# bjing2016/mdgen

Measured on AMD Instinct MI355X. Metric: sampled MD frames/sec, higher is better.
Workload: dtype bf16

## Files before the change

### mdgen_amd/csrc/api.hip

```cpp
#include "../../include/mdgen_amd.h"
#include "kernels.h"
#include "linear.h"

#include <algorithm>
#include <cmath>
#include <cstdarg>
#include <cstdio>
#include <cstdlib>
#include <cstring>
#include <climits>
#include <functional>
#include <map>
#include <string>
#include <vector>

using namespace mdg;

static thread_local char g_err[512] = "";
static int fail(int code, const char* fmt, ...) {
    va_list ap;
    va_start(ap, fmt);
    vsnprintf(g_err, sizeof(g_err), fmt, ap);
    va_end(ap);
    return code;
}
struct DryPlan {
    int view = -1;
    std::vector<std::pair<int, const char*>> rec;
};
static thread_local DryPlan* g_dry = nullptr;
#define HIPCHK(expr)                                                                           \
    do {                                                                                       \
        if (g_dry) break;                                                                      \
        hipError_t e_ = (expr);                                                                \
        if (e_ != hipSuccess) return fail((int)e_, "%s failed: %s", #expr, hipGetErrorString(e_)); \
    } while (0)
#define LAUNCHCHK()                                                                            \
    do {                                                                                       \
        hipError_t e_ = hipGetLastError();                                                     \
        if (e_ != hipSuccess) return fail((int)e_, "kernel launch failed: %s (%s:%d)", hipGetErrorString(e_), __FILE__, __LINE__); \
        if (const char* m_ = k32_take_launch_error()) return fail(-7, "internal: %s (%s:%d)", m_, __FILE__, __LINE__); \
    } while (0)

extern "C" const char* mdgen_last_error(void) { return g_err; }
extern "C" int32_t mdgen_abi_version(void) { return MDGEN_ABI_VERSION; }
extern "C" int32_t mdgen_dev_build(void) {
#ifdef MDGEN_DEV_BUILD
    return 1;
#else
    return 0;
#endif
}

constexpr int kMaxPos = 8160;
constexpr int kKS = 24;
constexpr size_t kPackCC = (size_t)12 * kKS * 64;

struct Lin { int w = -1, b = -1; };
struct MhaW {
    bf16x8 *wq = nullptr, *wk = nullptr, *wv_flash = nullptr, *wv_small = nullptr, *wo = nullptr;
    float *bq = nullptr, *bk = nullptr, *bv_flash = nullptr, *bv_small = nullptr, *bo = nullptr;
    float *bias_k = nullptr, *bias_v = nullptr;
    struct { Lin q, k, v, o; int bias_k = -1, bias_v = -1; } slot;
};
struct FfnW {
    bf16x8 *w1 = nullptr, *w2 = nullptr;
    float *b1 = nullptr, *b2 = nullptr;
    bf16x8* wstream = nullptr;
    float* w2f = nullptr;
    struct { Lin fc1, fc2; } slot;
};
struct TrunkW {
    MhaW mha_l, mha_t;
    FfnW ffn;
    Lin ada;
};
struct IpaW {
    float* gamma_beta = nullptr;
    bf16x8* wproj = nullptr;
    float* bproj = nullptr;
    float* head_w = nullptr;
    bf16x8* wout = nullptr;
    float* bout = nullptr;
    MhaW mha_l;
    FfnW ffn;
    struct { Lin ada, norm, q, kv, q_points, kv_points, out; int head_w = -1; } slot;
};

struct ProfRec {
    const char* cls;
    hipEvent_t a, b;
};

struct GraphEntry {
    std::vector<uint64_t> key;
    hipGraph_t graph = nullptr;
    hipGraphExec_t exec = nullptr;
};

struct WeightSlot {
    std::string name;
    std::function<int(const float*, const int64_t*, int, hipStream_t)> set;
    bool provided = false;
    float* f32 = nullptr;
    bool bound = false;
};

struct mdgen_ctx {
    mdgen_model_desc d;
    int nl = 0, D = 0, modrow = 0;
    std::vector<void*> allocs;
    std::vector<WeightSlot> weights;
    std::map<std::string, int> slot_of;
    struct { Lin latent, cond, t0, t2, rel_f, rel_r, fin, fin_ada; int mask = -1, aatype = -1; } slot;
    bool finalized = false;
    float *wl = nullptr, *bl = nullptr, *wc = nullptr, *bc = nullptr, *mask_emb = nullptr, *aa_emb = nullptr;
    float *wl_pack = nullptr, *wc_pack = nullptr;
    float* mask_delta = nullptr;
    bf16x8 *wl_hi = nullptr, *wl_lo = nullptr, *wc_hi = nullptr, *wc_lo = nullptr;
    float *pos_embed = nullptr, *t_w0 = nullptr, *t_b0 = nullptr, *t_w2 = nullptr, *t_b2 = nullptr;
    float *wf7 = nullptr, *bf7 = nullptr, *wr7 = nullptr, *br7 = nullptr;
    float *ada_w = nullptr, *ada_b = nullptr;
    float *inv_freq = nullptr, *rope = nullptr;
    bf16x8* wfin = nullptr;
    bf16x8* wfin_k = nullptr;
    float* bfin = nullptr;
    std::vector<TrunkW> trunk;
    std::vector<IpaW> ipa;
    int *map_nat = nullptr, *map_qk = nullptr, *map_vflash = nullptr, *map_vsmall = nullptr, *map_fin = nullptr;
    int *perm_qk = nullptr, *perm_vsmall = nullptr;
    int* mlp_tab = nullptr;
    std::vector<GraphEntry> graphs;
    bool inv_freq_set = false;
    bool prof_on = false;
    int opt_precision = 16;
    int opt_keep_fp32 = 0;
    int opt_streams = 2;
    bool opt_streams_auto = true;
    int opt_attn_path = 0;
    int opt_mlp_path = 1;
    int opt_fuse_proj_qkv = 1;
    int opt_fuse_proj = 3;
    int opt_panel_waves = 0;
    int ncu = 256;
    int opt_small_split = 1;
    bool xcd_round_robin = false;
    long n_split_launches = 0;
    int opt_flash_rotate = 1;
    int opt_flash_proj_form = 0;
    int opt_flash_proj = 1;
    int opt_train_precision = 32;
    int opt_train_streams = 2;
    hipStream_t train_side = nullptr;
    struct TurnReq { const float* w[3]; int nseg, rows, cols; size_t off; };
    std::vector<TurnReq> tr_plan;
    float* tr_buf = nullptr;
    size_t tr_buf_floats = 0;
    bool tr_plan_ok = false;
    std::vector<hipEvent_t> train_ev;
    size_t train_ev_next = 0;
    double* ode_host = nullptr;
    int opt_mlp_fold = 1;
    int opt_mlp_tail = 2;
    int opt_residue_l4 = 2;
    std::vector<void*> milestone_events;
    unsigned long long* phase_trace = nullptr;
    long phase_trace_cap = 0;
    std::vector<ProfRec> prof;
    static constexpr int kMaxSide = 7;
    hipStream_t side[kMaxSide] = {};
    hipEvent_t ev_fork = nullptr, ev_join[kMaxSide] = {};

    const float* f32(int slot) const { return weights[slot].f32; }
    bool any_f32() const {
        return std::any_of(weights.begin(), weights.end(), [](const WeightSlot& w) { return w.f32 != nullptr; });
    }
    template <typename T>
    int dalloc(T** p, size_t count) {
        void* q = nullptr;
        hipError_t e = hipMalloc(&q, count * sizeof(T));
        if (e != hipSuccess) return fail((int)e, "hipMalloc(%zu) failed: %s", count * sizeof(T), hipGetErrorString(e));
        allocs.push_back(q);
        *p = (T*)q;
        return 0;
    }
    int trunk_off(int i) const { return i * 9 * kC; }
    int ipa_off(int i) const { return nl * 9 * kC + i * 6 * kC; }
    int final_off() const { return nl * 15 * kC; }
};

static void decode_T(int rho, int& hd, int& h, int& e) {
    const int ft = rho / 32, m = rho % 32;
    const int b = m & 3, hh = (m >> 2) & 1, a = m >> 3;
    const int ap = 4 * ft + a;
    hd = ap / 3;
    h = hh;
    e = 4 * (ap % 3) + b;
}
static int feat_qk(int w, int rho) {
    int hd, h, e;
    decode_T(rho, hd, h, e);
    return (4 * w + hd) * kDH + 6 * h + (e >> 1) + 12 * (e & 1);
}
static int feat_vsmall(int w, int rho) {
    int hd, h, e;
    decode_T(rho, hd, h, e);
    return (4 * w + hd) * kDH + 12 * h + e;
}
static int feat_vflash(int w, int col) {
    const int hd = col / kDH, d = col % kDH;
    return (4 * w + hd) * kDH + 12 * ((d >> 2) & 1) + 4 * (d >> 3) + (d & 3);
}

static void build_maps(std::vector<int>& qk, std::vector<int>& vf, std::vector<int>& vs, std::vector<int>& pqk,
                       std::vector<int>& pvs) {
    qk.assign(kC, 0); vf.assign(kC, 0); vs.assign(kC, 0); pqk.assign(kC, 0); pvs.assign(kC, 0);
    for (int w = 0; w < 4; ++w)
        for (int r = 0; r < 96; ++r) {
            qk[w * 96 + r] = feat_qk(w, r);
            vs[w * 96 + r] = feat_vsmall(w, r);
            vf[w * 96 + r] = feat_vflash(w, r);
        }
    for (int w = 0; w < 4; ++w)
        for (int h = 0; h < 2; ++h)
            for (int hd = 0; hd < 4; ++hd)
                for (int e = 0; e < 12; ++e) {
                    const int i = ((w * 2 + h) * 4 + hd) * 12 + e;
                    pqk[i] = (4 * w + hd) * kDH + 6 * h + (e >> 1) + 12 * (e & 1);
                    pvs[i] = (4 * w + hd) * kDH + 12 * h + e;
                }
}

extern "C" int32_t mdgen_debug_layout_maps(int32_t* map_qk, int32_t* map_vflash, int32_t* map_vsmall,
                                           int32_t* perm_qk, int32_t* perm_vsmall) {
    if (!map_qk || !map_vflash || !map_vsmall || !perm_qk || !perm_vsmall) return fail(-1, "null argument");
    std::vector<int> qk, vf, vs, pqk, pvs;
    build_maps(qk, vf, vs, pqk, pvs);
    for (int i = 0; i < kC; ++i) {
        map_qk[i] = qk[i]; map_vflash[i] = vf[i]; map_vsmall[i] = vs[i]; perm_qk[i] = pqk[i]; perm_vsmall[i] = pvs[i];
    }
    return 0;
}

static std::vector<int> mlp_stream_table() {
    std::vector<int> t;
    auto xblock = [&](int c, int kx) {
        for (int q = 0; q < 12; ++q) t.push_back(0 << 16 | (2 * c + (q & 1)) << 8 | (6 * kx + (q >> 1)));
    };
    auto yblock = [&](int c, int kk) {
        for (int ft = 0; ft < 12; ++ft) t.push_back(1 << 16 | ft << 8 | (4 * c + kk));
    };
    for (int c = 0; c < 2; ++c)
        for (int kx = 0; kx < 4; ++kx) xblock(c, kx);
    for (int c = 1; c < 23; ++c)
        for (int b = 0; b < 4; ++b) {
            xblock(c + 1, b);
            yblock(c - 1, b);
        }
    for (int c = 22; c < 24; ++c)
        for (int kk = 0; kk < 4; ++kk) yblock(c, kk);
    return t;
}
constexpr int kMlpFrags = 2304;
extern "C" int32_t mdgen_debug_mlp_stream_table(int32_t* out, int32_t capacity) {
    const std::vector<int> t = mlp_stream_table();
    if (!out || capacity < (int)t.size()) return fail(-1, "need room for %d entries", (int)t.size());
    for (size_t i = 0; i < t.size(); ++i) out[i] = t[i];
    return (int32_t)t.size();
}

static int upload_ints(mdgen_ctx* c, int** dst, const std::vector<int>& v) {
    if (int r = c->dalloc(dst, v.size())) return r;
    HIPCHK(hipMemcpy(*dst, v.data(), v.size() * sizeof(int), hipMemcpyHostToDevice));
    return 0;
}

static bool shape_is(const int64_t* s, int nd, std::initializer_list<int64_t> want) {
    std::vector<int64_t> a(s, s + nd), b(want);
    while (a.size() > b.size() && a.front() == 1) a.erase(a.begin());
    return a == b;
}

static int add_weight(mdgen_ctx* c, const std::string& key, std::function<int(const float*, const int64_t*, int, hipStream_t)> set) {
    c->slot_of[key] = (int)c->weights.size();
    c->weights.push_back(WeightSlot{key, std::move(set)});
    return (int)c->weights.size() - 1;
}
#define SETTER(key, body)                                                                          \
    add_weight(c, key, [=](const float* data, const int64_t* shp, int nd, hipStream_t s) -> int {  \
        (void)shp; (void)nd; body; return 0; })
#define WANT(...) \
    if (!shape_is(shp, nd, {__VA_ARGS__})) return fail(-3, "unexpected shape for weight")

static int copy_f32(float* dst, const float* src, size_t n, hipStream_t s) {
    HIPCHK(hipMemcpyAsync(dst, src, n * sizeof(float), hipMemcpyDeviceToDevice, s));
    return 0;
}

static int register_mha(mdgen_ctx* c, const std::string& pre, MhaW* m) {
    const float qscale = (1.0f / std::sqrt((float)kDH)) * kLog2e;
    if (int r = c->dalloc(&m->wq, kPackCC)) return r;
    if (int r = c->dalloc(&m->wk, kPackCC)) return r;
    if (int r = c->dalloc(&m->wv_flash, kPackCC)) return r;
    if (int r = c->dalloc(&m->wv_small, kPackCC)) return r;
    if (int r = c->dalloc(&m->wo, kPackCC)) return r;
    for (float** p : {&m->bq, &m->bk, &m->bv_flash, &m->bv_small, &m->bo, &m->bias_k, &m->bias_v})
        if (int r = c->dalloc(p, (size_t)kC)) return r;
    m->slot.q.w = SETTER(pre + "q_proj.weight", {
        WANT(kC, kC);
        launch_pack_rows(data, kC, c->map_qk, 12, kKS, qscale, m->wq, s);
    });
    m->slot.q.b = SETTER(pre + "q_proj.bias", { WANT(kC); launch_gather_f32(data, c->perm_qk, qscale, m->bq, kC, s); });
    m->slot.k.w = SETTER(pre + "k_proj.weight", {
        WANT(kC, kC);
        launch_pack_rows(data, kC, c->map_qk, 12, kKS, 1.f, m->wk, s);
    });
    m->slot.k.b = SETTER(pre + "k_proj.bias", { WANT(kC); launch_gather_f32(data, c->perm_qk, 1.f, m->bk, kC, s); });
    m->slot.v.w = SETTER(pre + "v_proj.weight", {
        WANT(kC, kC);
        launch_pack_rows(data, kC, c->map_vflash, 12, kKS, 1.f, m->wv_flash, s);
        launch_pack_rows(data, kC, c->map_vsmall, 12, kKS, 1.f, m->wv_small, s);
    });
    m->slot.v.b = SETTER(pre + "v_proj.bias", {
        WANT(kC);
        launch_gather_f32(data, c->map_vflash, 1.f, m->bv_flash, kC, s);
        launch_gather_f32(data, c->perm_vsmall, 1.f, m->bv_small, kC, s);
    });
    m->slot.o.w = SETTER(pre + "out_proj.weight", {
        WANT(kC, kC);
        launch_pack_rows(data, kC, c->map_nat, 12, kKS, 1.f, m->wo, s);
    });
    m->slot.o.b = SETTER(pre + "out_proj.bias", { WANT(kC); if (int r = copy_f32(m->bo, data, kC, s)) return r; });
    m->slot.bias_k = SETTER(pre + "bias_k", { WANT(kC); if (int r = copy_f32(m->bias_k, data, kC, s)) return r; });
    m->slot.bias_v = SETTER(pre + "bias_v", { WANT(kC); if (int r = copy_f32(m->bias_v, data, kC, s)) return r; });
    SETTER(pre + "rot_emb.inv_freq", {
        WANT(12);
        if (int r = copy_f32(c->inv_freq, data, 12, s)) return r;
        c->inv_freq_set = true;
    });
    return 0;
}

static int register_ffn(mdgen_ctx* c, const std::string& pre, FfnW* f, bool trunk) {
    if (trunk)
        if (int r = c->dalloc(&f->w2f, (size_t)kC * kF)) return r;
    if (int r = c->dalloc(&f->w1, (size_t)48 * kKS * 64)) return r;
    if (int r = c->dalloc(&f->w2, (size_t)12 * 96 * 64)) return r;
    if (int r = c->dalloc(&f->b1, (size_t)kF)) return r;
    if (int r = c->dalloc(&f->b2, (size_t)kC)) return r;
    if (int r = c->dalloc(&f->wstream, (size_t)kMlpFrags * 64)) return r;
    f->slot.fc1.w = SETTER(pre + "fc1.weight", {
        WANT(kF, kC);
        launch_pack_rows(data, kC, c->map_nat, 48, kKS, 1.f, f->w1, s);
        launch_pack_stream(data, kC, 0, c->mlp_tab, kMlpFrags, 1.f, 1, f->wstream, s);
    });
    f->slot.fc1.b = SETTER(pre + "fc1.bias", { WANT(kF); if (int r = copy_f32(f->b1, data, kF, s)) return r; });
    f->slot.fc2.w = SETTER(pre + "fc2.weight", {
        WANT(kC, kF);
        launch_pack_rows(data, kF, c->map_nat, 12, 96, 1.f, f->w2, s);
        launch_pack_stream(data, kF, 1, c->mlp_tab, kMlpFrags, 1.f, 1, f->wstream, s);
        if (f->w2f)
            if (int r = copy_f32(f->w2f, data, (size_t)kC * kF, s)) return r;
    });
    f->slot.fc2.b = SETTER(pre + "fc2.bias", { WANT(kC); if (int r = copy_f32(f->b2, data, kC, s)) return r; });
    return 0;
}

extern "C" int32_t mdgen_ctx_create(mdgen_ctx** out, const mdgen_model_desc* d) {
    if (!out || !d) return fail(-1, "null argument");
    if (d->embed_dim != kC || d->mha_heads != kH) return fail(-2, "this build supports embed_dim=384, mha_heads=16 only");
    if (d->ipa_heads != 4 || d->ipa_head_dim != 32 || d->ipa_qk != 8 || d->ipa_v != 8)
        return fail(-2, "this build supports ipa_heads=4, ipa_head_dim=32, ipa_qk=ipa_v=8 only");
    if (d->num_layers < 1 || d->num_layers > 8) return fail(-2, "num_layers must be in 1..8");
    if (d->latent_dim != 21 && d->latent_dim != 28)
        return fail(-2, "latent_dim must be 21 (forward simulation) or 28 (two-sided conditioning)");
    if (d->tps_condition && d->latent_dim != 28) return fail(-2, "tps_condition requires latent_dim 28");
    int ndev = 0;
    HIPCHK(hipGetDeviceCount(&ndev));
    if (ndev < 1) return fail(-9, "no HIP device");
    mdgen_ctx* c = new mdgen_ctx();
    {
        int dev = 0, ncu = 0;
        if (hipGetDevice(&dev) == hipSuccess && hipDeviceGetAttribute(&ncu, hipDeviceAttributeMultiprocessorCount, dev) == hipSuccess && ncu > 0)
            c->ncu = ncu;
    }
    {
        int* dp = nullptr;
        int hx[64];
        hipStream_t ps = nullptr;
        if (hipStreamCreateWithFlags(&ps, hipStreamNonBlocking) == hipSuccess) {
            if (hipMalloc((void**)&dp, sizeof(hx)) == hipSuccess) {
                launch_xcc_probe(dp, 64, ps);
                if (hipGetLastError() == hipSuccess &&
                    hipMemcpyAsync(hx, dp, sizeof(hx), hipMemcpyDeviceToHost, ps) == hipSuccess &&
                    hipStreamSynchronize(ps) == hipSuccess) {
                    bool ok = true;
                    for (int i = 8; i < 64; ++i) ok = ok && hx[i] == hx[i & 7];
                    c->xcd_round_robin = ok;
                }
                (void)hipFree(dp);
            }
            (void)hipStreamDestroy(ps);
        }
        (void)hipGetLastError();
    }
    c->d = *d;
    c->nl = d->num_layers;
    c->D = d->latent_dim;
    c->modrow = (15 * c->nl + 2) * kC;
    const int D = c->D, nl = c->nl;
    std::vector<int> nat(kF), qk, vf, vs, fin(32), pqk, pvs;
    for (int i = 0; i < kF; ++i) nat[i] = i;
    build_maps(qk, vf, vs, pqk, pvs);
    for (int i = 0; i < 32; ++i) fin[i] = i < D ? i : -1;
#define TRY(x) do { if (int r_ = (x)) { mdgen_ctx_destroy(c); return r_; } } while (0)
    TRY(upload_ints(c, &c->map_nat, nat));
    TRY(upload_ints(c, &c->map_qk, qk));
    TRY(upload_ints(c, &c->map_vflash, vf));
    TRY(upload_ints(c, &c->map_vsmall, vs));
    TRY(upload_ints(c, &c->map_fin, fin));
    TRY(upload_ints(c, &c->mlp_tab, mlp_stream_table()));
    TRY(upload_ints(c, &c->perm_qk, pqk));
    TRY(upload_ints(c, &c->perm_vsmall, pvs));
    TRY(c->dalloc(&c->wl, (size_t)kC * D));
    TRY(c->dalloc(&c->wl_pack, (size_t)kEmbPackFloats));
    TRY(c->dalloc(&c->wc_pack, (size_t)kEmbPackFloats));
    TRY(c->dalloc(&c->mask_delta, (size_t)kC));
    for (bf16x8** q : {&c->wl_hi, &c->wl_lo, &c->wc_hi, &c->wc_lo}) TRY(c->dalloc(q, (size_t)12 * 2 * 64));
    TRY(c->dalloc(&c->bl, (size_t)kC));
    TRY(c->dalloc(&c->wc, (size_t)kC * D));
    TRY(c->dalloc(&c->bc, (size_t)kC));
    TRY(c->dalloc(&c->mask_emb, (size_t)2 * kC));
    TRY(c->dalloc(&c->aa_emb, (size_t)21 * kC));
    TRY(c->dalloc(&c->t_w0, (size_t)kC * 256));
    TRY(c->dalloc(&c->t_b0, (size_t)kC));
    TRY(c->dalloc(&c->t_w2, (size_t)kC * kC));
    TRY(c->dalloc(&c->t_b2, (size_t)kC));
    TRY(c->dalloc(&c->ada_w, (size_t)c->modrow * kC));
    TRY(c->dalloc(&c->ada_b, (size_t)c->modrow));
    TRY(c->dalloc(&c->inv_freq, (size_t)12));
    TRY(c->dalloc(&c->rope, (size_t)(kMaxPos + 1) * kRopeRow));
#define TRYHIP(expr)                                                                                    \
    do {                                                                                                \
        hipError_t e_ = (expr);                                                                         \
        if (e_ != hipSuccess) {                                                                         \
            mdgen_ctx_destroy(c);                                                                       \
            return fail((int)e_, "%s failed: %s", #expr, hipGetErrorString(e_));                        \
        }                                                                                               \
    } while (0)
    for (int i = 0; i < mdgen_ctx::kMaxSide; ++i) {
        TRYHIP(hipStreamCreateWithFlags(&c->side[i], hipStreamNonBlocking));
        TRYHIP(hipEventCreateWithFlags(&c->ev_join[i], hipEventDisableTiming));
    }
    TRYHIP(hipEventCreateWithFlags(&c->ev_fork, hipEventDisableTiming));
    TRY(c->dalloc(&c->wfin, (size_t)kKS * 64));
    TRY(c->dalloc(&c->wfin_k, (size_t)kKS * 64));
    TRY(c->dalloc(&c->bfin, (size_t)32));
    TRYHIP(hipMemset(c->bfin, 0, 32 * sizeof(float)));
#undef TRYHIP
    c->slot.latent.w = SETTER("latent_to_emb.weight", { WANT(kC, c->D); if (int r = copy_f32(c->wl, data, (size_t)kC * c->D, s)) return r; launch_pack_embed(c->wl, c->D, c->wl_pack, s);
        launch_pack_rows(c->wl, c->D, c->map_nat, 12, 2, 1.f, c->wl_hi, s, 1, 0); launch_pack_rows(c->wl, c->D, c->map_nat, 12, 2, 1.f, c->wl_lo, s, 1, 1); });
    c->slot.latent.b = SETTER("latent_to_emb.bias", { WANT(kC); if (int r = copy_f32(c->bl, data, kC, s)) return r; });
    c->slot.cond.w = SETTER("cond_to_emb.weight", { WANT(kC, c->D); if (int r = copy_f32(c->wc, data, (size_t)kC * c->D, s)) return r; launch_pack_embed(c->wc, c->D, c->wc_pack, s);
        launch_pack_rows(c->wc, c->D, c->map_nat, 12, 2, 1.f, c->wc_hi, s, 1, 0); launch_pack_rows(c->wc, c->D, c->map_nat, 12, 2, 1.f, c->wc_lo, s, 1, 1); });
    c->slot.cond.b = SETTER("cond_to_emb.bias", { WANT(kC); if (int r = copy_f32(c->bc, data, kC, s)) return r; });
    c->slot.mask = SETTER("mask_to_emb.weight", { WANT(2, kC); if (int r = copy_f32(c->mask_emb, data, 2 * kC, s)) return r; launch_sub_f32(c->mask_emb + kC, c->mask_emb, c->mask_delta, kC, s); });
    c->slot.aatype = SETTER("aatype_to_emb.weight", { WANT(21, kC); if (int r = copy_f32(c->aa_emb, data, 21 * kC, s)) return r; });
    c->slot.t0.w = SETTER("t_embedder.mlp.0.weight", { WANT(kC, 256); if (int r = copy_f32(c->t_w0, data, (size_t)kC * 256, s)) return r; });
    c->slot.t0.b = SETTER("t_embedder.mlp.0.bias", { WANT(kC); if (int r = copy_f32(c->t_b0, data, kC, s)) return r; });
    c->slot.t2.w = SETTER("t_embedder.mlp.2.weight", { WANT(kC, kC); if (int r = copy_f32(c->t_w2, data, (size_t)kC * kC, s)) return r; });
    c->slot.t2.b = SETTER("t_embedder.mlp.2.bias", { WANT(kC); if (int r = copy_f32(c->t_b2, data, kC, s)) return r; });
    if (d->abs_pos_emb) {
        if (d->crop < 1) { mdgen_ctx_destroy(c); return fail(-2, "abs_pos_emb requires crop >= 1"); }
        TRY(c->dalloc(&c->pos_embed, (size_t)d->crop * kC));
        SETTER("pos_embed", { WANT(c->d.crop, kC); if (int r = copy_f32(c->pos_embed, data, (size_t)c->d.crop * kC, s)) return r; });
    }
    if (d->tps_condition) {
        TRY(c->dalloc(&c->wf7, (size_t)kC * 7));
        TRY(c->dalloc(&c->bf7, (size_t)kC));
        TRY(c->dalloc(&c->wr7, (size_t)kC * 7));
        TRY(c->dalloc(&c->br7, (size_t)kC));
        c->slot.rel_f.w = SETTER("latent_to_emb_f.weight", { WANT(kC, 7); if (int r = copy_f32(c->wf7, data, kC * 7, s)) return r; });
        c->slot.rel_f.b = SETTER("latent_to_emb_f.bias", { WANT(kC); if (int r = copy_f32(c->bf7, data, kC, s)) return r; });
        c->slot.rel_r.w = SETTER("latent_to_emb_r.weight", { WANT(kC, 7); if (int r = copy_f32(c->wr7, data, kC * 7, s)) return r; });
        c->slot.rel_r.b = SETTER("latent_to_emb_r.bias", { WANT(kC); if (int r = copy_f32(c->br7, data, kC, s)) return r; });
    }
    c->slot.fin.w = SETTER("emb_to_latent.linear.weight",
           { WANT(c->D, kC); launch_pack_rows(data, kC, c->map_fin, 1, kKS, 1.f, c->wfin, s); launch_pack_rows(data, kC, c->map_fin, 1, kKS, 1.f, c->wfin_k, s, 1); });
    c->slot.fin.b = SETTER("emb_to_latent.linear.bias", { WANT(c->D); if (int r = copy_f32(c->bfin, data, c->D, s)) return r; });
    c->slot.fin_ada.w = SETTER("emb_to_latent.adaLN_modulation.1.weight", {
        WANT(2 * kC, kC);
        if (int r = copy_f32(c->ada_w + (size_t)c->final_off() * kC, data, (size_t)2 * kC * kC, s)) return r;
    });
    c->slot.fin_ada.b = SETTER("emb_to_latent.adaLN_modulation.1.bias",
           { WANT(2 * kC); if (int r = copy_f32(c->ada_b + c->final_off(), data, 2 * kC, s)) return r; });
    c->trunk.resize(nl);
    c->ipa.resize(nl);
    for (int i = 0; i < nl; ++i) {
        const std::string p = "layers." + std::to_string(i) + ".";
        TrunkW* t = &c->trunk[i];
        t->ada.w = SETTER(p + "adaLN_modulation.1.weight", {
            WANT(9 * kC, kC);
            if (int r = copy_f32(c->ada_w + (size_t)c->trunk_off(i) * kC, data, (size_t)9 * kC * kC, s)) return r;
        });
        t->ada.b = SETTER(p + "adaLN_modulation.1.bias",
               { WANT(9 * kC); if (int r = copy_f32(c->ada_b + c->trunk_off(i), data, 9 * kC, s)) return r; });
        TRY(register_mha(c, p + "mha_t.attn.", &t->mha_t));
        TRY(register_mha(c, p + "mha_l.attn.", &t->mha_l));
        TRY(register_ffn(c, p, &t->ffn, true));
    }
    for (int i = 0; i < nl; ++i) {
        const std::string p = "ipa_layers." + std::to_string(i) + ".";
        IpaW* w = &c->ipa[i];
        TRY(c->dalloc(&w->gamma_beta, (size_t)2 * kC));
        TRY(c->dalloc(&w->wproj, (size_t)21 * kKS * 64));
        TRY(c->dalloc(&w->bproj, (size_t)kIpaProj));
        TRY(c->dalloc(&w->head_w, (size_t)4));
        TRY(c->dalloc(&w->wout, (size_t)12 * 16 * 64));
        TRY(c->dalloc(&w->bout, (size_t)kC));
        w->slot.ada.w = SETTER(p + "adaLN_modulation.1.weight", {
            WANT(6 * kC, kC);
            if (int r = copy_f32(c->ada_w + (size_t)c->ipa_off(i) * kC, data, (size_t)6 * kC * kC, s)) return r;
        });
        w->slot.ada.b = SETTER(p + "adaLN_modulation.1.bias",
               { WANT(6 * kC); if (int r = copy_f32(c->ada_b + c->ipa_off(i), data, 6 * kC, s)) return r; });
        w->slot.norm.w = SETTER(p + "ipa_norm.weight", { WANT(kC); if (int r = copy_f32(w->gamma_beta, data, kC, s)) return r; });
        w->slot.norm.b = SETTER(p + "ipa_norm.bias", { WANT(kC); if (int r = copy_f32(w->gamma_beta + kC, data, kC, s)) return r; });
        w->slot.head_w = SETTER(p + "ipa.head_weights", { WANT(4); if (int r = copy_f32(w->head_w, data, 4, s)) return r; });
        w->slot.q.w = SETTER(p + "ipa.linear_q.weight", { WANT(128, kC); launch_pack_rows(data, kC, c->map_nat, 4, kKS, 1.f, w->wproj, s); });
        w->slot.q.b = SETTER(p + "ipa.linear_q.bias", { WANT(128); if (int r = copy_f32(w->bproj, data, 128, s)) return r; });
        w->slot.kv.w = SETTER(p + "ipa.linear_kv.weight",
               { WANT(256, kC); launch_pack_rows(data, kC, c->map_nat, 8, kKS, 1.f, w->wproj + (size_t)4 * kKS * 64, s); });
        w->slot.kv.b = SETTER(p + "ipa.linear_kv.bias", { WANT(256); if (int r = copy_f32(w->bproj + 128, data, 256, s)) return r; });
        w->slot.q_points.w = SETTER(p + "ipa.linear_q_points.weight",
               { WANT(96, kC); launch_pack_rows(data, kC, c->map_nat, 3, kKS, 1.f, w->wproj + (size_t)12 * kKS * 64, s); });
        w->slot.q_points.b = SETTER(p + "ipa.linear_q_points.bias", { WANT(96); if (int r = copy_f32(w->bproj + 384, data, 96, s)) return r; });
        w->slot.kv_points.w = SETTER(p + "ipa.linear_kv_points.weight",
               { WANT(192, kC); launch_pack_rows(data, kC, c->map_nat, 6, kKS, 1.f, w->wproj + (size_t)15 * kKS * 64, s); });
        w->slot.kv_points.b = SETTER(p + "ipa.linear_kv_points.bias", { WANT(192); if (int r = copy_f32(w->bproj + 480, data, 192, s)) return r; });
        w->slot.out.w = SETTER(p + "ipa.linear_out.weight",
               { WANT(kC, kIpaFeat); launch_pack_rows(data, kIpaFeat, c->map_nat, 12, 16, 1.f, w->wout, s); });
        w->slot.out.b = SETTER(p + "ipa.linear_out.bias", { WANT(kC); if (int r = copy_f32(w->bout, data, kC, s)) return r; });
        TRY(register_mha(c, p + "mha_l.attn.", &w->mha_l));
        TRY(register_ffn(c, p, &w->ffn, false));
    }
#undef TRY
    *out = c;
    return 0;
}

extern "C" int32_t mdgen_ctx_destroy(mdgen_ctx* c) {
    if (!c) return 0;
    for (auto& g : c->graphs) {
        if (g.exec) (void)hipGraphExecDestroy(g.exec);
        if (g.graph) (void)hipGraphDestroy(g.graph);
    }
    if (c->ev_fork) (void)hipEventDestroy(c->ev_fork);
    for (hipEvent_t e : c->train_ev) (void)hipEventDestroy(e);
    if (c->train_side) (void)hipStreamDestroy(c->train_side);
    if (c->tr_buf) (void)hipFree(c->tr_buf);
    if (c->ode_host) (void)hipHostFree(c->ode_host);
    for (int i = 0; i < mdgen_ctx::kMaxSide; ++i) {
        if (c->ev_join[i]) (void)hipEventDestroy(c->ev_join[i]);
        if (c->side[i]) (void)hipStreamDestroy(c->side[i]);
    }
    for (void* p : c->allocs) (void)hipFree(p);
    delete c;
    return 0;
}

extern "C" int32_t mdgen_ctx_num_weights(const mdgen_ctx* c) { return c ? (int32_t)c->weights.size() : 0; }
extern "C" const char* mdgen_ctx_weight_name(const mdgen_ctx* c, int32_t i) {
    if (!c || i < 0 || i >= (int32_t)c->weights.size()) return nullptr;
    return c->weights[i].name.c_str();
}

extern "C" int32_t mdgen_ctx_set_weight(mdgen_ctx* c, const char* key, const float* data, const int64_t* shape,
                                        int32_t ndim, void* stream) {
    if (!c || !key || !data || !shape) return fail(-1, "null argument");
    auto it = c->slot_of.find(key);
    if (it == c->slot_of.end()) return fail(-4, "unknown weight key '%s'", key);
    WeightSlot& w = c->weights[it->second];
    const int r = w.set(data, shape, ndim, (hipStream_t)stream);
    if (r) {
        if (r == -3) {
            char buf[160] = "";
            int o = 0;
            for (int i = 0; i < ndim && o < 140; ++i) o += snprintf(buf + o, sizeof(buf) - o, "%lld,", (long long)shape[i]);
            return fail(-3, "unexpected shape (%s) for weight '%s'", buf, key);
        }
        return r;
    }
    LAUNCHCHK();
    if (c->opt_keep_fp32) {
        size_t n = 1;
        for (int i = 0; i < ndim; ++i) n *= (size_t)shape[i];
        if (!w.f32)
            if (int e = c->dalloc(&w.f32, n)) return e;
        if (w.f32 != data && !w.bound)
            HIPCHK(hipMemcpyAsync(w.f32, data, n * sizeof(float), hipMemcpyDeviceToDevice, (hipStream_t)stream));
    }
    w.provided = true;
    c->finalized = false;
    return 0;
}

extern "C" int32_t mdgen_ctx_finalize(mdgen_ctx* c, void* stream) {
    if (!c) return fail(-1, "null context");
    for (const WeightSlot& w : c->weights)
        if (!w.provided) return fail(-5, "weight '%s' was not provided", w.name.c_str());
    if (!c->inv_freq_set) return fail(-5, "rot_emb.inv_freq was not provided");
    launch_rope_table(c->rope, c->inv_freq, kMaxPos + 1, (hipStream_t)stream);
    LAUNCHCHK();
    c->finalized = true;
    return 0;
}

extern "C" int32_t mdgen_ctx_set_option(mdgen_ctx* c, const char* name, int32_t value) {
    if (!c || !name) return fail(-1, "null argument");
    const std::string n(name);
    if (n == "streams") {
        if (value < 1 || value > mdgen_ctx::kMaxSide + 1) return fail(-2, "streams must be in 1..%d", mdgen_ctx::kMaxSide + 1);
        c->opt_streams = value;
        c->opt_streams_auto = false;
    } else if (n == "keep_fp32_weights") {
        if (value != 0 && value != 1) return fail(-2, "keep_fp32_weights must be 0 or 1");
        c->opt_keep_fp32 = value;
    } else if (n == "precision") {
        if (value != 16 && value != 32) return fail(-2, "precision must be 16 (bf16 operands) or 32 (fp32 operands)");
        if (value == 32 && (!c->opt_keep_fp32 || !c->any_f32()))
            return fail(-6, "precision 32 needs the fp32 weight copies: set option keep_fp32_weights = 1 before loading weights");
        c->opt_precision = value;
    } else if (n == "attention_path") {
        if (value != 0 && value != 1) return fail(-2, "attention_path must be 0 (auto) or 1 (robust loop always)");
        c->opt_attn_path = value;
    } else if (n == "fuse_proj") {
        if (value != 0 && value != 3) return fail(-2, "fuse_proj must be 0 (off) or 3 (inside the panel MLP kernel where that kernel runs)");
        c->opt_fuse_proj = value;
    } else if (n == "fuse_proj_qkv") {
        if (value != 0 && value != 1) return fail(-2, "fuse_proj_qkv must be 0 or 1");
        c->opt_fuse_proj_qkv = value;
    } else if (n == "small_split") {
        if (value != 0 && value != 1) return fail(-2, "small_split must be 0 or 1");
        c->opt_small_split = value;
    } else if (n == "panel_waves") {
        if (value != 0 && value != 4 && value != 8) return fail(-2, "panel_waves must be 0 (by launch size), 4 or 8");
        c->opt_panel_waves = value;
    } else if (n == "flash_rotate") {
        if (value != 0 && value != 1) return fail(-2, "flash_rotate must be 0 or 1");
        c->opt_flash_rotate = value;
    } else if (n == "flash_proj_form") {
        if (value != 0 && value != 4 && value != 8) return fail(-2, "flash_proj_form must be 0 (by shape), 4 or 8");
        c->opt_flash_proj_form = value;
    } else if (n == "flash_proj") {
        if (value < 0 || value > 2) return fail(-2, "flash_proj must be 0 (off), 1 (launches that fill the chip) or 2 (always)");
        c->opt_flash_proj = value;
    } else if (n == "mlp_path") {
        if (value < 0 || value > 2) return fail(-2, "mlp_path must be 0 (panel kernel), 1 (row-owner kernel when it fills the chip) or 2 (always)");
        c->opt_mlp_path = value;
    } else if (n == "train_precision") {
        if (value != 16 && value != 32) return fail(-2, "train_precision must be 32 (fp32 operands, exact) or 16 (bf16 operands, fp32 accumulate)");
        c->opt_train_precision = value;
    } else if (n == "train_streams") {
        if (value != 1 && value != 2) return fail(-2, "train_streams must be 1 (one stream) or 2 (weight gradients on a second stream)");
        c->opt_train_streams = value;
    } else if (n == "mlp_fold") {
        if (value != 0 && value != 1) return fail(-2, "mlp_fold must be 0 or 1");
        c->opt_mlp_fold = value;
    } else if (n == "mlp_tail") {
        if (value < 0 || value > 2) return fail(-2, "mlp_tail must be 0 (off), 1 (FinalLayer + Euler update) or 2 (... + the next step's token embedding)");
        c->opt_mlp_tail = value;
    } else if (n == "residue_l4_path") {
        if (value < 0 || value > 2) return fail(-2, "residue_l4_path must be 0, 1 or 2");
        c->opt_residue_l4 = value;
    } else {
        return fail(-4, "unknown option '%s'", name);
    }
    return 0;
}

static size_t align256(size_t x) { return (x + 255) & ~(size_t)255; }

static long split_panels(const mdgen_ctx* c, long maxrows) {
    if (!c->opt_small_split) return 0;
    const long pn = (maxrows + kPanel - 1) / kPanel, cap = c->ncu / kMlpSplit < kMlpSplitMaxPanels ? c->ncu / kMlpSplit : kMlpSplitMaxPanels;
    return pn < cap ? pn : cap;
}
constexpr size_t kSplitCounterBytes = 1024;
static_assert(kMlpSplitMaxPanels * sizeof(unsigned) <= kSplitCounterBytes, "counter block");
static size_t split_bytes(long panels) { return kSplitCounterBytes + 2 * (size_t)panels * kMlpSplit * kPanel * kC * 4; }

static bool mlp_uses_rows(const mdgen_ctx* c, long nrows) {
    const long tiles = (nrows + 31) / 32;
    return c->opt_mlp_path == 2 || (c->opt_mlp_path == 1 && tiles >= 3L * c->ncu);
}
constexpr size_t kFoldStreamBytes = (size_t)kMlpFrags * 1024;
constexpr size_t kFoldMaxBytes = (size_t)8 << 30;
static size_t fold_bytes(const mdgen_ctx* c, int S) { return (size_t)S * c->nl * (kFoldStreamBytes + (size_t)kC * 4); }
static bool fold_on(const mdgen_ctx* c, long nrows, int t_shared, int S) {
    return t_shared && c->opt_mlp_fold && c->opt_precision == 16 && mlp_uses_rows(c, nrows) && fold_bytes(c, S) <= kFoldMaxBytes;
}
static bool embed_base_on(const mdgen_ctx* c, long nrows, int t_shared, int S) {
    return fold_on(c, nrows, t_shared, S) && c->opt_mlp_tail == 2 && S > 1;
}

static size_t frag_bytes(long nseq, int len) { return (size_t)nseq * kH * (len / 32 + 1) * kFragBytes; }

constexpr long kMaxViewTokens = 0xFFFFFFFFL / (kC * 4);

static int plan_views(long B, long T, long L, int streams) {
    const long tl = T * L;
    if (tl > kMaxViewTokens) return 0;
    const long per = kMaxViewTokens / tl;
    long nv = (B + per - 1) / per;
    if (nv < streams) nv = streams;
    if (nv > B) nv = B;
    while ((B + nv - 1) / nv > per) ++nv;
    return (int)nv;
}

extern "C" int32_t mdgen_debug_view_plan(const mdgen_shape* sh, int32_t streams, int32_t* n_views,
                                         int32_t* max_batch_per_view) {
    if (!sh || !n_views || !max_batch_per_view) return fail(-1, "null argument");
    if (sh->B < 1 || sh->T < 1 || sh->L < 1 || streams < 1) return fail(-2, "B, T, L, streams must be >= 1");
    const int nv = plan_views(sh->B, sh->T, sh->L, streams);
    if (nv == 0) return fail(-2, "one sample (T*L = %ld tokens) exceeds the per-launch limit of %ld tokens",
                             (long)sh->T * sh->L, kMaxViewTokens);
    *n_views = nv;
    *max_batch_per_view = (sh->B + nv - 1) / nv;
    return 0;
}

static int check_shape(const mdgen_ctx* c, const mdgen_shape* sh, int S) {
    if (!c || !sh) return fail(-1, "null argument");
    if (sh->B < 1 || sh->T < 1 || sh->L < 1 || S < 1) return fail(-2, "B, T, L, n_steps must be >= 1");
    if (sh->T > kMaxPos - 1 || sh->L > kMaxPos - 1) return fail(-2, "T and L must be < %d", kMaxPos - 1);
    if ((long)sh->B * sh->T * sh->L > 1500000000L) return fail(-2, "token count too large");
    if ((long)sh->T * sh->L > kMaxViewTokens)
        return fail(-2, "one sample (T*L = %ld tokens) exceeds the per-launch limit of %ld tokens", (long)sh->T * sh->L,
                    kMaxViewTokens);
    if ((long)S * sh->B * sh->L > kMaxViewTokens)
        return fail(-2, "n_steps*B*L = %ld rows of the IPA table exceed the per-launch limit of %ld", (long)S * sh->B * sh->L,
                    kMaxViewTokens);
    if (c->d.abs_pos_emb && sh->L > c->d.crop) return fail(-2, "L=%d exceeds pos_embed crop=%d", sh->L, c->d.crop);
    return 0;
}

extern "C" int32_t mdgen_workspace_layout(const mdgen_ctx* c, const mdgen_shape* sh, int32_t S, int32_t t_shared,
                                          mdgen_ws_layout* o) {
    if (!o) return fail(-1, "null argument");
    if (int r = check_shape(c, sh, S)) return r;
    const long B = sh->B, T = sh->T, L = sh->L;
    const long N = B * T * L, Mp = (long)S * B * L, R = t_shared ? S : (long)S * B;
    const long maxrows = N > Mp ? N : Mp;
    size_t fq = (size_t)maxrows * 3 * kC * 2;
    size_t fkv = 0;
    auto upd = [&](size_t b) { if (b > fq) fq = b; if (b > fkv) fkv = b; };
    upd(frag_bytes(B * L, (int)T));
    if (L > 8) {
        upd(frag_bytes(B * T, (int)L));
        upd(frag_bytes((long)S * B, (int)L));
    }
    if (fkv == 0) fkv = 256;
    size_t off = 0;
    auto take = [&](size_t bytes) { size_t a = off; off += align256(bytes); return a; };
// ... 232 lines not shown
    switch (f) {
    case MlpPanelForm::W4: return trunk ? "mlp@p4" : "ipa.mlp@p4";
    case MlpPanelForm::W8: return trunk ? "mlp@p8" : "ipa.mlp@p8";
    case MlpPanelForm::W8Split: return trunk ? "mlp@p8x3" : "ipa.mlp@p8x3";
    case MlpPanelForm::PreW4: return trunk ? "proj_mlp@p4" : "ipa.mlp@p4";
    case MlpPanelForm::PreW8: return trunk ? "proj_mlp@p8" : "ipa.mlp@p8";
    case MlpPanelForm::PreW8Split: return trunk ? "proj_mlp@p8x3" : "ipa.mlp@p8x3";
    }
    return nullptr;
}

static int panel_waves_for(const mdgen_ctx* c, long panels) {
    return c->opt_panel_waves == 4 || c->opt_panel_waves == 8 ? c->opt_panel_waves : (panels <= c->ncu ? 8 : 4);
}
static QkvForm qkv_form(const mdgen_ctx* c, const AxisMap& ax) {
    const long panels = (long)ax.nseq * ((ax.len + kPanel - 1) / kPanel);
    if (panel_waves_for(c, panels) != 8) return QkvForm::Panel4;
    if (!c->opt_small_split || 2 * panels > c->ncu) return QkvForm::Panel8;
    return 2L * ax.nseq * ((ax.len + 31) / 32) <= c->ncu ? QkvForm::Panel8SplitHalf : QkvForm::Panel8Split;
}
static Attn4Form attn4_fused_form(const mdgen_ctx* c, long nrows) {
#ifdef MDGEN_DEV_ATTN4_FULL
    return Attn4Form::Fused;
#else
    return c->opt_small_split && (nrows + 31) / 32 <= c->ncu ? Attn4Form::FusedHalf : Attn4Form::Fused;
#endif
}
static bool flash_proj_on(const mdgen_ctx* c, const AxisMap& ax) {
    return c->opt_precision == 16 && (c->opt_flash_proj == 2 || (c->opt_flash_proj == 1 && flash_proj_jobs(ax) >= 2L * c->ncu));
}
static FlashProjForm flash_proj_form(const mdgen_ctx* c, const AxisMap& ax) {
    const long jobs8 = (long)ax.nseq * ((ax.len + 2 * kPanel - 1) / (2 * kPanel));
    const int w = c->opt_flash_proj_form ? c->opt_flash_proj_form : (ax.len >= 512 && jobs8 >= c->ncu) ? 8 : 4;
    return w == 8 ? FlashProjForm::Q128 : FlashProjForm::Q64;
}

enum class AttnPath { Quad, Micro, Tiled };
enum class ProjAt { Own, Attention, NextQkv, Mlp };
struct AttnPlan {
    Pos pos;
    AttnPath path;
    Attn4Form a4;
    QkvForm qkv;
    bool flash_proj;
    FlashProjForm fp;
    ProjAt proj;
};
static AttnPlan attn_plan(const mdgen_ctx* c, Pos pos, const AxisMap& ax, long nrows, bool pre, ProjAt later) {
    AttnPlan a{pos, AttnPath::Tiled, Attn4Form::AttnOnly, QkvForm::Small, false, FlashProjForm::Q64, ProjAt::Own};
    const bool small = pos != Pos::TimeT && ax.len <= 8;
    if (small && ax.len == 4 && c->opt_residue_l4 != 0) {
        a.path = AttnPath::Quad;
        if (c->opt_residue_l4 == 2) {
            a.a4 = attn4_fused_form(c, nrows);
            a.proj = ProjAt::Attention;
        }
    } else if (small) {
        a.path = AttnPath::Micro;
    } else {
        a.qkv = pre ? QkvForm::PreProj : qkv_form(c, ax);
        a.flash_proj = flash_proj_on(c, ax);
        a.fp = flash_proj_form(c, ax);
        a.proj = a.flash_proj ? ProjAt::Attention : later;
    }
    return a;
}

struct MlpPlan {
    bool trunk, use_rows;
    MlpRowsForm rows;
    MlpPanelForm panel;
};
static MlpPlan mlp_plan(const mdgen_ctx* c, bool trunk, long nrows, bool pre, MlpRowsForm rows, bool concurrent, long split_cap, bool trace) {
    MlpPlan m{trunk, !pre && mlp_uses_rows(c, nrows), rows, MlpPanelForm::W4};
    if (m.use_rows) return m;
    const long panels = (nrows + kPanel - 1) / kPanel;
    const int pw = trace ? 4 : panel_waves_for(c, panels);
    const bool split = pw == 8 && c->opt_small_split && c->xcd_round_robin && !concurrent && panels * kMlpSplit <= c->ncu && panels <= split_cap;
    m.panel = split ? (pre ? MlpPanelForm::PreW8Split : MlpPanelForm::W8Split)
              : pw == 8 ? (pre ? MlpPanelForm::PreW8 : MlpPanelForm::W8)
                        : (pre ? MlpPanelForm::PreW4 : MlpPanelForm::W4);
    return m;
}

struct LayerPlan {
    AttnPlan l, t;
    MlpPlan mlp;
};
static bool embed_tail_runs(const Run& r) { return r.fold_ready && mlp_uses_rows(r.c, r.N) && r.c->opt_mlp_tail && r.embase_p; }
static LayerPlan layer_plan(const Run& r, const AxisMap& axL, const AxisMap& axT, bool last, bool embed_next, bool trace) {
    const mdgen_ctx* c = r.c;
    LayerPlan p;
    const MlpRowsForm rows = !r.fold_ready                   ? MlpRowsForm::Plain
                             : !(last && c->opt_mlp_tail)    ? MlpRowsForm::Fold
                             : embed_next                    ? MlpRowsForm::FoldFinalEmbed
                                                             : MlpRowsForm::FoldFinal;
    const bool fuse_lt = c->opt_fuse_proj_qkv && r.L > 8 && r.T > 8;
    p.l = attn_plan(c, Pos::ResL, axL, r.N, false, fuse_lt ? ProjAt::NextQkv : ProjAt::Own);
    const bool fuse = c->opt_fuse_proj == 3 && !mlp_uses_rows(c, r.N);
    p.t = attn_plan(c, Pos::TimeT, axT, r.N, p.l.proj == ProjAt::NextQkv, fuse ? ProjAt::Mlp : ProjAt::Own);
    p.mlp = mlp_plan(c, true, r.N, p.t.proj == ProjAt::Mlp, rows, r.concurrent, r.split_cap, trace);
    return p;
}

struct Rows {
    float* h;
    long nrows;
    ModMap mm;
    int chunk0;
};
struct OutProj {
    const bf16x8* w;
    const float* bias;
    int gate_chunk;
};

static int attn_sublayer(const Run& r, const AttnPlan& pl, const MhaW& m, const Rows& rw, const AxisMap& ax, const MaskMap& mk,
                         const OutProj& pre) {
    if (int e = check_launch_rows(rw.nrows)) return e;
    const int gate = rw.chunk0 + 2;
    QkvParams q{};
    q.h = rw.h;
    q.nrows = rw.nrows;
    q.ax = ax;
    q.mm = rw.mm;
    q.shift_chunk = rw.chunk0;
    q.scale_chunk = rw.chunk0 + 1;
    q.wq = m.wq;
    q.wk = m.wk;
    q.bq = m.bq;
    q.bk = m.bk;
    q.rope = r.c->rope;
    q.qf = r.qfp;
    q.kf = r.kfp;
    q.vf = r.vfp;
    q.qkv_small = (__bf16*)r.qfp;
    const int ppanel = pl.qkv == QkvForm::Panel8SplitHalf ? 32 : kPanel;
    q.panels_per_seq = (ax.len + ppanel - 1) / ppanel;
    ProjParams p{};
    p.h = rw.h;
    p.nrows = rw.nrows;
    p.mm = rw.mm;
    p.gate_chunk = gate;
    p.gated = 1;
    p.w = m.wo;
    p.bias = m.bo;
    p.a_bf16 = r.obufp;
    switch (pl.path) {
    case AttnPath::Quad:
        q.wv = m.wv_small;
        q.bv = m.bv_small;
        q.bias_k = m.bias_k;
        q.bias_v = m.bias_v;
        q.mk = mk;
        q.obuf = r.obufp;
        if (pl.proj == ProjAt::Attention) {
            q.h_rw = rw.h;
            q.wo = m.wo;
            q.bo = m.bo;
            q.gate_chunk = gate;
        }
        if (int e = launch(r, tag(pl.pos, pl.a4), [&] { launch_ln_qkv_attn4(q, pl.a4, r.s); })) return e;
        break;
    case AttnPath::Micro:
        q.wv = m.wv_small;
        q.bv = m.bv_small;
        if (int e = launch(r, tag(pl.pos, pl.qkv), [&] { launch_ln_qkv(q, pl.qkv, r.s); })) return e;
        p.a_bf16 = nullptr;
        p.qkv_small = q.qkv_small;
        p.ax = ax;
        p.mk = mk;
        p.bias_k = m.bias_k;
        p.bias_v = m.bias_v;
        p.rope = r.c->rope;
        return launch(r, tag_proj(pl.pos), [&] { launch_proj(p, ProjMode::MicroAttn, r.s); });
    case AttnPath::Tiled: {
        q.wv = m.wv_flash;
        q.bv = m.bv_flash;
        q.bias_k = m.bias_k;
        q.bias_v = m.bias_v;
        q.mk = mk;
        q.vmask = (uint32_t*)(q.vf + flash_vmask_offset(ax.nseq, ax.ntile()));
        q.vmask_stride = flash_vmask_stride(ax.ntile());
        if (pl.qkv == QkvForm::PreProj) {
            q.obuf = r.obufp;
            q.wo = pre.w;
            q.bo = pre.bias;
            q.gate_chunk = pre.gate_chunk;
            q.h_rw = rw.h;
        }
        if (int e = launch(r, tag(pl.pos, pl.qkv), [&] { launch_ln_qkv(q, pl.qkv, r.s); })) return e;
        FlashParams f{};
        f.ax = ax;
        f.mk = mk;
        f.qf = q.qf;
        f.kf = q.kf;
        f.vf = q.vf;
        f.bias_k = m.bias_k;
        f.bias_v = m.bias_v;
        f.rope = r.c->rope;
        f.obuf = r.obufp;
        f.force_robust = r.c->opt_attn_path;
        f.rotate = r.c->opt_flash_rotate;
        f.vmask = q.vmask;
        f.vmask_stride = q.vmask_stride;
        if (pl.flash_proj) {
            FlashProjParams fp{};
            fp.f = f;
            fp.h = rw.h;
            fp.mm = rw.mm;
            fp.gate_chunk = gate;
            fp.wo = m.wo;
            fp.bo = m.bo;
            return launch(r, tag(pl.pos, pl.fp), [&] { launch_flash_proj(fp, pl.fp, r.s); });
        }
        if (int e = launch(r, tag_flash(pl.pos), [&] { launch_flash(f, r.s); })) return e;
        break;
    }
    }
    if (pl.proj != ProjAt::Own) return 0;
    return launch(r, tag_proj(pl.pos), [&] { launch_proj(p, ProjMode::Plain, r.s); });
}

struct MlpTrunk {
    long fold_sl;
    const FinalParams* fin;
    int next_step;
    unsigned long long* trace;
    long trace_cap;
};
static int mlp_sublayer(const Run& r, const MlpPlan& pl, const FfnW& f, const Rows& rw, const OutProj& pre, const MlpTrunk* tk) {
    if (int e = check_launch_rows(rw.nrows)) return e;
    if (pl.use_rows) {
        MlpRowsParams q{};
        q.h = rw.h;
        q.nrows = rw.nrows;
        q.mm = rw.mm;
        q.shift_chunk = rw.chunk0;
        q.scale_chunk = rw.chunk0 + 1;
        q.gate_chunk = rw.chunk0 + 2;
        q.wstream = (const unsigned char*)f.wstream;
        q.b1 = f.b1;
        q.b2 = f.b2;
        if (pl.rows != MlpRowsForm::Plain) {
            q.wstream = r.fold_streams + (size_t)tk->fold_sl * kFoldStreamBytes;
            q.b2g = r.fold_b2g + (size_t)tk->fold_sl * kC;
        }
        if (pl.rows == MlpRowsForm::FoldFinal || pl.rows == MlpRowsForm::FoldFinalEmbed) {
            const FinalParams* tail = tk->fin;
            q.tail_w = r.c->wfin_k;
            q.tail_b = tail->bias;
            q.tail_mod = tail->mm.mod;
            q.tail_D = tail->D;
            q.tail_euler = tail->euler;
            q.tail_dt = tail->dt;
            q.tail_x = tail->x;
            q.tail_out = tail->out;
        }
        if (pl.rows == MlpRowsForm::FoldFinalEmbed) {
            q.emb_wl_hi = r.c->wl_hi;
            q.emb_wl_lo = r.c->wl_lo;
            q.emb_wc_hi = r.c->wc_hi;
            q.emb_wc_lo = r.c->wc_lo;
            q.emb_base = r.embase_p + (long)tk->next_step * r.embase_step_stride;
            q.emb_mdelta = r.c->mask_delta;
            q.emb_xcond = r.x_cond;
            q.emb_cmask = r.x_cond_mask;
            q.emb_T = r.T;
            q.emb_L = r.L;
        }
        if (tk && tk->trace) {
            q.trace = tk->trace;
            q.trace_cap = tk->trace_cap;
        }
        return launch(r, tag(pl.trunk, pl.rows), [&] { launch_mlp_rows(q, pl.rows, r.s); });
    }
    MlpParams p{};
    const bool fused = pl.panel == MlpPanelForm::PreW4 || pl.panel == MlpPanelForm::PreW8 || pl.panel == MlpPanelForm::PreW8Split;
    if (fused) {
        p.o = r.obufp;
        p.wo = pre.w;
        p.bo = pre.bias;
        p.gate_chunk_o = pre.gate_chunk;
    }
    p.h = rw.h;
    p.nrows = rw.nrows;
    p.mm = rw.mm;
    p.shift_chunk = rw.chunk0;
    p.scale_chunk = rw.chunk0 + 1;
    p.gate_chunk = rw.chunk0 + 2;
    p.w1 = f.w1;
    p.w2 = f.w2;
    p.b1 = f.b1;
    p.b2 = f.b2;
    if (tk && tk->trace) {
        p.trace = tk->trace;
        p.trace_cap = tk->trace_cap;
    }
    if (pl.panel == MlpPanelForm::W8Split || pl.panel == MlpPanelForm::PreW8Split) {
        ++r.c->n_split_launches;
        p.part = r.split_part;
        p.hupd = r.split_hupd;
        p.counters = r.split_counters;
    }
    return launch(r, tag(pl.trunk, pl.panel), [&] { launch_mlp(p, pl.panel, r.s); });
}
// ... 765 lines not shown
```

### mdgen_amd/csrc/k_gemm.hip

```cpp
#include "kernels.h"
#include "panel.h"

namespace mdg {

constexpr int kRowB = kC * 2;
constexpr int kPanelBytes = kPanel * kRowB;

template <bool ROPE, int TT = 2>
__device__ __forceinline__ void epilogue_heads_T(const f32x16* acc , const PanelRows* pr, int w,
                                                 const float* __restrict__ bias_perm, const float* __restrict__ rope,
                                                 bool small, int pos0, int len, int seq, int ntile, int tile0,
                                                 unsigned char* __restrict__ frag, __bf16* __restrict__ small_dst,
                                                 int which) {
    const int lane = lane_id(), hh = lane >> 5, tk = lane & 31;
    f32x4 bq[4][3];
    {
        const f32x4* bp = reinterpret_cast<const f32x4*>(bias_perm + (w * 2 + hh) * 48);
#pragma unroll
        for (int hd = 0; hd < 4; ++hd)
#pragma unroll
            for (int c = 0; c < 3; ++c) bq[hd][c] = bp[hd * 3 + c];
    }
    int tokv[TT], posv[TT];
    f32x4 rq[TT][4];
#pragma unroll
    for (int tt = 0; tt < TT; ++tt) {
        const int row = tt * 32 + tk;
        tokv[tt] = pr->tok[row];
        int pos = small ? (tokv[tt] >= 0 ? tokv[tt] % len : 0) : pos0 + row;
        if (pos > len) pos = len;
        posv[tt] = pos;
        if (ROPE) {
            const f32x4* rc = reinterpret_cast<const f32x4*>(rope + (long)pos * kRopeRow + 16 * hh);
#pragma unroll
            for (int i = 0; i < 4; ++i) rq[tt][i] = rc[i];
        }
    }
#pragma unroll
    for (int tt = 0; tt < TT; ++tt) {
        const int token = tokv[tt];
        const bool valid = token >= 0;
        float cs[6], sn[6];
        if (ROPE) {
#pragma unroll
            for (int p = 0; p < 6; ++p) {
                cs[p] = rq[tt][p >> 2][p & 3];
                sn[p] = rq[tt][2 + (p >> 2)][p & 3];
            }
        }
        const int tile = tile0 + tt;
#pragma unroll
        for (int hd = 0; hd < 4; ++hd) {
            float e[12];
#pragma unroll
            for (int c = 0; c < 3; ++c) {
                const int ap = 3 * hd + c, ft = ap >> 2, a = ap & 3;
#pragma unroll
                for (int b = 0; b < 4; ++b) e[4 * c + b] = acc[ft * TT + tt][4 * a + b] + bq[hd][c][b];
            }
            if (ROPE) {
#pragma unroll
                for (int p = 0; p < 6; ++p) {
                    const float x1 = e[2 * p], x2 = e[2 * p + 1];
                    e[2 * p] = x1 * cs[p] - x2 * sn[p];
                    e[2 * p + 1] = x2 * cs[p] + x1 * sn[p];
                }
            }
            uint32_t u[6];
#pragma unroll
            for (int i = 0; i < 6; ++i) u[i] = pack_bf16(e[2 * i], e[2 * i + 1]);
            const int head = 4 * w + hd;
            if (small) {
                if (valid) {
                    u32x2* d = reinterpret_cast<u32x2*>(small_dst + (long)token * (3 * kC) + which * kC + head * kDH + hh * 12);
                    d[0] = u32x2{u[0], u[1]};
                    d[1] = u32x2{u[2], u[3]};
                    d[2] = u32x2{u[4], u[5]};
                }
            } else if (tile < ntile) {
                if (which == 1) {
                    unsigned char* base = frag + ((long)(seq * kH + head) * ntile + tile) * kFragK;
                    *reinterpret_cast<u32x4*>(base + lane * 16) = u32x4{u[0], u[1], u[2], u[3]};
                    *reinterpret_cast<u32x4*>(base + 1024 + lane * 16) = u32x4{u[4], u[5], 0x3f803f80u, 0u};
                } else {
                    unsigned char* base = frag + ((long)(seq * kH + head) * ntile + tile) * kFragQ;
                    *reinterpret_cast<u32x4*>(base + lane * 16) = u32x4{u[0], u[1], u[2], u[3]};
                    *reinterpret_cast<u32x2*>(base + 1024 + lane * 8) = u32x2{u[4], u[5]};
                }
            }
        }
    }
}

template <int TT = 2>
__device__ __forceinline__ void epilogue_v_flash(const f32x16* acc , int w,
                                                 const float* __restrict__ bias_perm, int seq, int ntile, int tile0,
                                                 unsigned char* __restrict__ vf) {
    const int lane = lane_id(), hh = lane >> 5, n = lane & 31;
#pragma unroll
    for (int j = 0; j < 3; ++j) {
        const int col = 32 * j + n;
        const int hd = col / kDH, d = col - hd * kDH;
        const float b = bias_perm[w * 96 + col];
        const int head = 4 * w + hd;
#pragma unroll
        for (int tt = 0; tt < TT; ++tt) {
            const int tile = tile0 + tt;
            if (tile < ntile) {
                unsigned char* base = vf + ((long)(seq * kH + head) * ntile + tile) * kFragV + hh * 400 + d * 16;
                const f32x16 a = acc[tt * 3 + j];
                *reinterpret_cast<u32x4*>(base) = u32x4{pack_bf16(a[0] + b, a[1] + b), pack_bf16(a[2] + b, a[3] + b),
                                                         pack_bf16(a[4] + b, a[5] + b), pack_bf16(a[6] + b, a[7] + b)};
                *reinterpret_cast<u32x4*>(base + 800) =
                    u32x4{pack_bf16(a[8] + b, a[9] + b), pack_bf16(a[10] + b, a[11] + b),
                          pack_bf16(a[12] + b, a[13] + b), pack_bf16(a[14] + b, a[15] + b)};
            }
        }
    }
    if (lane < 32) {
        const int hd = lane & 3, tt = (lane >> 2) & 1, h2 = (lane >> 3) & 1, ks = lane >> 4;
        const int tile = tile0 + tt;
        if (tt < TT && tile < ntile)
            *reinterpret_cast<u32x4*>(vf + ((long)(seq * kH + 4 * w + hd) * ntile + tile) * kFragV + ks * 800 + h2 * 400 + kDH * 16) =
                u32x4{0x3f803f80u, 0x3f803f80u, 0x3f803f80u, 0x3f803f80u};
    }
}

__device__ __forceinline__ void write_bias_slots(const QkvParams& p, int seq, int w, bool do_k = true, bool do_v = true, int tpp = 2) {
    const int lane = lane_id();
    const int len = p.ax.len, nt = p.ax.ntile();
    const int kt = len >> 5, sl = len & 31;
    if (kt >= tpp * p.panels_per_seq) {
#pragma unroll
        for (int hd = 0; hd < 4; ++hd) {
            const long ft = (long)(seq * kH + 4 * w + hd) * nt + kt;
            u32x4* kd = reinterpret_cast<u32x4*>(p.kf + ft * kFragK);
            u32x4* vd = reinterpret_cast<u32x4*>(p.vf + ft * kFragV);
            const u32x4 z = {0u, 0u, 0u, 0u}, ones = {0x3f803f80u, 0x3f803f80u, 0x3f803f80u, 0x3f803f80u};
            if (do_k) {
                kd[lane] = z;
                kd[64 + lane] = u32x4{0u, 0u, 0x3f803f80u, 0u};
            }
            const int r0 = lane, r1 = 64 + lane;
            if (do_v) {
                vd[r0] = (r0 % 25) == kDH ? ones : z;
                if (r1 < 100) vd[r1] = (r1 % 25) == kDH ? ones : z;
            }
        }
        __builtin_amdgcn_sched_barrier(0);
    }
    if (do_k && lane < 8) {
        const int hd = lane & 3, hh = lane >> 2, head = 4 * w + hd;
        const float* bk = p.bias_k + head * kDH;
        const float* rc = p.rope + (long)len * kRopeRow + 16 * hh;
        float e[12];
#pragma unroll
        for (int pp = 0; pp < 6; ++pp) {
            const int i = 6 * hh + pp;
            const float x1 = bk[i], x2 = bk[i + 12], c = rc[pp], sn = rc[8 + pp];
            e[2 * pp] = x1 * c - x2 * sn;
            e[2 * pp + 1] = x2 * c + x1 * sn;
        }
        unsigned char* base = p.kf + ((long)(seq * kH + head) * nt + kt) * kFragK;
        *reinterpret_cast<u32x4*>(base + (hh * 32 + sl) * 16) =
            u32x4{pack_bf16(e[0], e[1]), pack_bf16(e[2], e[3]), pack_bf16(e[4], e[5]), pack_bf16(e[6], e[7])};
        *reinterpret_cast<u32x4*>(base + 1024 + (hh * 32 + sl) * 16) =
            u32x4{pack_bf16(e[8], e[9]), pack_bf16(e[10], e[11]), 0x3f803f80u, 0u};
    }
    if (do_v && lane < kDH) {
        const int d = lane;
        const int dpsi = 12 * ((d >> 2) & 1) + 4 * (d >> 3) + (d & 3);
        const int hk = (sl >> 2) & 1, r = (sl & 3) + 4 * (sl >> 3);
#pragma unroll
        for (int hd = 0; hd < 4; ++hd) {
            const int head = 4 * w + hd;
            unsigned char* base = p.vf + ((long)(seq * kH + head) * nt + kt) * kFragV;
            const uint32_t v = pack_bf16(p.bias_v[head * kDH + dpsi], 0.f);
            *reinterpret_cast<uint16_t*>(base + (r >> 3) * 800 + hk * 400 + d * 16 + (r & 7) * 2) = (uint16_t)v;
        }
    }
}

#ifdef MDGEN_DEV_QKV_STAMPS
__device__ unsigned long long g_qkv_stamps[16384 * 8];
extern "C" int mdgen_dev_qkv_stamps(void* host, size_t bytes) {
    return (int)hipMemcpyFromSymbol(host, HIP_SYMBOL(g_qkv_stamps), bytes);
}
#define QKV_STAMP(slot)                                                                                      \
    if (!SMALL && lane_id() == 0 && (long)blockIdx.x * 4 + wave_id() < 16384)                                  \
    g_qkv_stamps[((long)blockIdx.x * 4 + wave_id()) * 8 + (slot)] = __builtin_amdgcn_s_memtime()
__device__ unsigned long long g_attn4_stamps[8192 * 16];
extern "C" int mdgen_dev_attn4_stamps(void* host, size_t bytes) {
    return (int)hipMemcpyFromSymbol(host, HIP_SYMBOL(g_attn4_stamps), bytes);
}
#define ATTN4_STAMP_DECL unsigned long long a4st[11] = {}
#define ATTN4_STAMP(slot)                          \
    a4st[slot] = __builtin_amdgcn_s_memtime();     \
    __builtin_amdgcn_sched_barrier(0)
#define ATTN4_STAMP_FLUSH                                                                                   \
    if (lane_id() == 0 && (long)blockIdx.x * 4 + wave_id() < 8192) {                                          \
        _Pragma("unroll") for (int k = 0; k < 11; ++k)                                                        \
            g_attn4_stamps[((long)blockIdx.x * 4 + wave_id()) * 16 + k] = a4st[k];                            \
    }
#else
#define QKV_STAMP(slot)
#define ATTN4_STAMP_DECL
#define ATTN4_STAMP(slot)
#define ATTN4_STAMP_FLUSH
#endif

template <bool SMALL, bool PRE = false>
__global__ __launch_bounds__(256, 2) void k_ln_qkv(const QkvParams p) {
    __shared__ __attribute__((aligned(16))) unsigned char smem[sizeof(PanelRows) + kPanelBytes];
    PanelRows* pr = reinterpret_cast<PanelRows*>(smem);
    unsigned char* panel = smem + sizeof(PanelRows);
    int seq = 0, pos0 = 0, tile0 = 0;
    if (SMALL) {
        setup_rows_linear(pr, (long)blockIdx.x * kPanel, p.nrows, p.mm);
    } else {
        seq = blockIdx.x / p.panels_per_seq;
        const int pn = blockIdx.x - seq * p.panels_per_seq;
        pos0 = pn * kPanel;
        tile0 = pn * 2;
        setup_rows_axis(pr, p.ax, seq, pos0, p.mm);
        if (wave_id() == 0) {
            const int lane = lane_id(), len = p.ax.len, pos = pos0 + lane;
            const float mv = p.mk.at(p.ax.token(seq, pos < len ? pos : len - 1));
            const unsigned long long bal = __ballot(pos == len || (pos < len && mv != 0.f));
            uint32_t* vm = p.vmask + (long)seq * p.vmask_stride;
            if (lane < 2) vm[tile0 + lane] = (uint32_t)(bal >> (32 * lane));
            if (pn == p.panels_per_seq - 1) {
                const int idx = tile0 + 2 + lane;
                if (idx < p.vmask_stride) vm[idx] = idx == (len >> 5) ? 1u << (len & 31) : 0u;
                if (idx + 64 < p.vmask_stride) vm[idx + 64] = 0u;
            }
        }
    }
    QKV_STAMP(0);
    __syncthreads();
    const int w = __builtin_amdgcn_readfirstlane(wave_id()), lane = lane_id();
    f32x16 acc[6];
    if (PRE) {
        prologue_bf16<kC>(panel, pr, p.obuf);
        __syncthreads();
        zero_acc<6>(acc);
        wave_gemm<2, 3, 24, false>(panel, kRowB, 0, 0, p.wo + (size_t)(3 * w) * 24 * 64 + lane, 24 * 64, acc);
        __syncthreads();
        epilogue_gate_residual_lds<3>(acc, pr, reinterpret_cast<float*>(panel) + w * (32 * 96), 96 * w, p.bo, p.mm, p.gate_chunk,
                                      true, p.h_rw);
        __syncthreads();
    }
    prologue_ln<false>(panel, pr, PRE ? p.h_rw : p.h, p.mm, p.shift_chunk, p.scale_chunk, 1e-6f);
    __syncthreads();
    QKV_STAMP(1);
    const int ntile = p.ax.ntile();
    const int len = p.ax.len;
    zero_acc<6>(acc);
    wave_gemm<2, 3, 24, true>(panel, kRowB, 0, 0, p.wq + (size_t)(3 * w) * 24 * 64 + lane, 24 * 64, acc);
    QKV_STAMP(2);
    epilogue_heads_T<true>(acc, pr, w, p.bq, p.rope, SMALL, pos0, len, seq, ntile, tile0, p.qf, p.qkv_small, 0);
    __builtin_amdgcn_sched_barrier(0);
    QKV_STAMP(3);
    zero_acc<6>(acc);
    wave_gemm<2, 3, 24, true>(panel, kRowB, 0, 0, p.wk + (size_t)(3 * w) * 24 * 64 + lane, 24 * 64, acc);
    QKV_STAMP(4);
    epilogue_heads_T<true>(acc, pr, w, p.bk, p.rope, SMALL, pos0, len, seq, ntile, tile0, p.kf, p.qkv_small, 1);
    __builtin_amdgcn_sched_barrier(0);
    QKV_STAMP(5);
    zero_acc<6>(acc);
    if (SMALL) {
        wave_gemm<2, 3, 24, true>(panel, kRowB, 0, 0, p.wv + (size_t)(3 * w) * 24 * 64 + lane, 24 * 64, acc);
        epilogue_heads_T<false>(acc, pr, w, p.bv, nullptr, true, pos0, len, seq, ntile, tile0, nullptr, p.qkv_small, 2);
    } else {
        wave_gemm<2, 3, 24, false>(panel, kRowB, 0, 0, p.wv + (size_t)(3 * w) * 24 * 64 + lane, 24 * 64, acc);
        QKV_STAMP(6);
        epilogue_v_flash(acc, w, p.bv, seq, ntile, tile0, p.vf);
        if ((int)blockIdx.x - seq * p.panels_per_seq == p.panels_per_seq - 1) {
            __builtin_amdgcn_sched_barrier(0);
            write_bias_slots(p, seq, w);
        }
        QKV_STAMP(7);
    }
}

template <int J>
__device__ __forceinline__ float quad_bcast(float v) {
    return __builtin_bit_cast(float, __builtin_amdgcn_update_dpp(0, __builtin_bit_cast(int, v), J * 0x55, 0xf, 0xf, true));
}
__device__ __forceinline__ float half_sum(float x) {
    const auto r = __builtin_amdgcn_permlane32_swap(__float_as_uint(x), __float_as_uint(x), false, false);
    return __uint_as_float(r[0]) + __uint_as_float(r[1]);
}
template <int TT = 2>
__device__ __forceinline__ void head_values(const f32x16* acc, int tt, int hd, const f32x4 (&bq)[3], float (&e)[12]) {
#pragma unroll
    for (int c = 0; c < 3; ++c) {
        const int ap = 3 * hd + c, ft = ap >> 2, a = ap & 3;
#pragma unroll
        for (int b = 0; b < 4; ++b) e[4 * c + b] = acc[ft * TT + tt][4 * a + b] + bq[c][b];
    }
}
__device__ __forceinline__ void load_head_bias(const float* bias_perm, int w, int hh, f32x4 (&bq)[4][3]) {
    const f32x4* bp = reinterpret_cast<const f32x4*>(bias_perm + (w * 2 + hh) * 48);
#pragma unroll
    for (int hd = 0; hd < 4; ++hd)
#pragma unroll
        for (int c = 0; c < 3; ++c) bq[hd][c] = bp[hd * 3 + c];
}


template <bool SPLIT, bool HALF = false>
__global__ __launch_bounds__(512, 1) void k_ln_qkv8(const QkvParams p) {
    static_assert(!HALF || SPLIT, "32-row workgroups exist in the split form only");
    constexpr int TT = HALF ? 1 : 2, kRows = 32 * TT;
    __shared__ __attribute__((aligned(16))) unsigned char smem[sizeof(PanelRows) + kPanelBytes];
    PanelRows* pr = reinterpret_cast<PanelRows*>(smem);
    unsigned char* panel = smem + sizeof(PanelRows);
    const int blk = SPLIT ? blockIdx.x >> 1 : blockIdx.x, half = SPLIT ? blockIdx.x & 1 : 0;
    const int seq = blk / p.panels_per_seq;
    const int pn = blk - seq * p.panels_per_seq;
    const int pos0 = pn * kRows, tile0 = pn * TT;
    setup_rows_axis(pr, p.ax, seq, pos0, p.mm, kRows);
    if (wave_id() == 0 && half == 0) {
        const int lane = lane_id(), len = p.ax.len, pos = pos0 + lane;
        const float mv = p.mk.at(p.ax.token(seq, pos < len ? pos : len - 1));
        const unsigned long long bal = __ballot(pos == len || (pos < len && mv != 0.f));
        uint32_t* vm = p.vmask + (long)seq * p.vmask_stride;
        if (lane < TT) vm[tile0 + lane] = (uint32_t)(bal >> (32 * lane));
        if (pn == p.panels_per_seq - 1) {
            const int idx = tile0 + TT + lane;
            if (idx < p.vmask_stride) vm[idx] = idx == (len >> 5) ? 1u << (len & 31) : 0u;
            if (idx + 64 < p.vmask_stride) vm[idx + 64] = 0u;
        }
    }
    __syncthreads();
    const int w8 = __builtin_amdgcn_readfirstlane(wave_id()), g = w8 >> 2, w = w8 & 3, lane = lane_id();
    if (HALF) {
        if (g == 0) prologue_ln<false, 0, 1>(panel, pr, p.h, p.mm, p.shift_chunk, p.scale_chunk, 1e-6f, w, lane);
        else prologue_ln<false, 1, 2>(panel, pr, p.h, p.mm, p.shift_chunk, p.scale_chunk, 1e-6f, w, lane);
    } else {
        if (g == 0) prologue_ln<false, 0, 2>(panel, pr, p.h, p.mm, p.shift_chunk, p.scale_chunk, 1e-6f, w, lane);
        else prologue_ln<false, 2, 4>(panel, pr, p.h, p.mm, p.shift_chunk, p.scale_chunk, 1e-6f, w, lane);
    }
    __syncthreads();
    const int ntile = p.ax.ntile(), len = p.ax.len;
    const bool last = pn == p.panels_per_seq - 1;
    f32x16 acc[3 * TT];
    const bool do_q = SPLIT ? half == 0 && g == 0 : g == 0, do_k = SPLIT ? half == 0 && g == 1 : g == 0;
    const bool do_v = SPLIT ? half == 1 && g == 0 : g == 1;
    if (do_q) {
        zero_acc<3 * TT>(acc);
        wave_gemm<TT, 3, 24, true>(panel, kRowB, 0, 0, p.wq + (size_t)(3 * w) * 24 * 64 + lane, 24 * 64, acc);
        epilogue_heads_T<true, TT>(acc, pr, w, p.bq, p.rope, false, pos0, len, seq, ntile, tile0, p.qf, p.qkv_small, 0);
        __builtin_amdgcn_sched_barrier(0);
    }
    if (do_k) {
        zero_acc<3 * TT>(acc);
        wave_gemm<TT, 3, 24, true>(panel, kRowB, 0, 0, p.wk + (size_t)(3 * w) * 24 * 64 + lane, 24 * 64, acc);
        epilogue_heads_T<true, TT>(acc, pr, w, p.bk, p.rope, false, pos0, len, seq, ntile, tile0, p.kf, p.qkv_small, 1);
        if (last) {
            __builtin_amdgcn_sched_barrier(0);
            write_bias_slots(p, seq, w, true, false, TT);
        }
    }
    if (do_v) {
        zero_acc<3 * TT>(acc);
        wave_gemm<TT, 3, 24, false>(panel, kRowB, 0, 0, p.wv + (size_t)(3 * w) * 24 * 64 + lane, 24 * 64, acc);
        epilogue_v_flash<TT>(acc, w, p.bv, seq, ntile, tile0, p.vf);
        if (last) {
            __builtin_amdgcn_sched_barrier(0);
            write_bias_slots(p, seq, w, false, true, TT);
        }
    }
}

constexpr int kAttn4KPF = 2, kAttn4VPF = 3;
template <bool PROJ, bool HALF = false>
__global__ __launch_bounds__(256, 2) void k_ln_qkv_attn4(const QkvParams p) {
    static_assert(!HALF || PROJ, "the half-panel form is the whole sub-layer");
    constexpr int TT = HALF ? 1 : 2, kRows = HALF ? 32 : kPanel;
    __shared__ __attribute__((aligned(16))) unsigned char smem[sizeof(PanelRows) + kPanelBytes];
    __shared__ uint32_t qstash[HALF ? 1 : 4][24][64];
    PanelRows* pr = reinterpret_cast<PanelRows*>(smem);
    unsigned char* panel = smem + sizeof(PanelRows);
    ATTN4_STAMP_DECL;
    ATTN4_STAMP(0);
    {
        const long row0 = (long)blockIdx.x * kRows, rend = row0 + kRows;
        setup_rows_linear(pr, row0, rend < p.nrows ? rend : p.nrows, p.mm);
    }
    __syncthreads();
    const int w = __builtin_amdgcn_readfirstlane(wave_id());
    constexpr int t0 = 0;
    if (HALF) prologue_ln<false, 0, 2>(panel, pr, p.h, p.mm, p.shift_chunk, p.scale_chunk, 1e-6f, w, lane_id());
    else prologue_ln<false>(panel, pr, p.h, p.mm, p.shift_chunk, p.scale_chunk, 1e-6f);
    __syncthreads();
    ATTN4_STAMP(1);
    const int lane = lane_id(), hh = lane >> 5, tk = lane & 31;
    constexpr int L = 4;
    int tok[TT];
    float mval[TT];
#pragma unroll
    for (int tt = 0; tt < TT; ++tt) {
        tok[tt] = pr->tok[(t0 + tt) * 32 + tk];
        mval[tt] = p.mk.at(tok[tt] < 0 ? 0 : tok[tt]);
    }
    auto load_rope = [&](f32x4 (&rq)[TT][4]) {
#pragma unroll
        for (int tt = 0; tt < TT; ++tt) {
            const int tc = tok[tt] < 0 ? 0 : tok[tt];
            const f32x4* rc = reinterpret_cast<const f32x4*>(p.rope + (long)(tc & (L - 1)) * kRopeRow + 16 * hh);
#pragma unroll
            for (int i = 0; i < 4; ++i) rq[tt][i] = rc[i];
        }
    };
    f32x16 acc[3 * TT];
    f32x4 bb[4][3];
    f32x4 rq[TT][4];
    zero_acc<3 * TT>(acc);
    wave_gemm<TT, 3, 24, true>(panel, kRowB, t0, 0, p.wq + (size_t)(3 * w) * 24 * 64 + lane, 24 * 64, acc);
    ATTN4_STAMP(2);
    load_head_bias(p.bq, w, hh, bb);
    load_rope(rq);
    uint32_t qp[TT][4][6];
#pragma unroll
    for (int tt = 0; tt < TT; ++tt)
#pragma unroll
        for (int hd = 0; hd < 4; ++hd) {
            float e[12];
            head_values<TT>(acc, tt, hd, bb[hd], e);
#pragma unroll
            for (int q = 0; q < 6; ++q) {
                const float c = rq[tt][q >> 2][q & 3], sn = rq[tt][2 + (q >> 2)][q & 3];
                const float x1 = e[2 * q], x2 = e[2 * q + 1];
                qp[tt][hd][q] = pack_bf16(x1 * c - x2 * sn, x2 * c + x1 * sn);
            }
        }
    if constexpr (!HALF) {
#pragma unroll
        for (int hd = 0; hd < 4; ++hd)
#pragma unroll
            for (int q = 0; q < 6; ++q) qstash[w][hd * 6 + q][lane] = qp[TT - 1][hd][q];
    }
    ATTN4_STAMP(3);
    __builtin_amdgcn_sched_barrier(0);
    zero_acc<3 * TT>(acc);
    wave_gemm<TT, 3, 24, true, HALF ? 4 : kAttn4KPF>(panel, kRowB, t0, 0, p.wk + (size_t)(3 * w) * 24 * 64 + lane, 24 * 64, acc);
    ATTN4_STAMP(4);
    load_head_bias(p.bk, w, hh, bb);
    load_rope(rq);
#pragma unroll
    for (int tt = 0; tt < TT; ++tt)
#pragma unroll
        for (int hd = 0; hd < 4; ++hd) {
            float k[12];
            head_values<TT>(acc, tt, hd, bb[hd], k);
#pragma unroll
            for (int c = 0; c < 3; ++c) {
                const int ap = 3 * hd + c, ft = ap >> 2, a = ap & 3;
#pragma unroll
                for (int b2 = 0; b2 < 2; ++b2) {
                    const int q = 2 * c + b2;
                    const float cs = rq[tt][q >> 2][q & 3], sn = rq[tt][2 + (q >> 2)][q & 3];
                    const float x1 = k[2 * q], x2 = k[2 * q + 1];
                    acc[ft * TT + tt][4 * a + 2 * b2] = x1 * cs - x2 * sn;
                    acc[ft * TT + tt][4 * a + 2 * b2 + 1] = x2 * cs + x1 * sn;
                }
            }
        }
    ATTN4_STAMP(5);
    __builtin_amdgcn_sched_barrier(0);
    float P[TT][4][5];
    {
        const float* rcL = p.rope + (long)L * kRopeRow + 16 * hh;
#pragma unroll
        for (int hd = 0; hd < 4; ++hd) {
            const float* bk = p.bias_k + (4 * w + hd) * kDH;
            float kb[12];
#pragma unroll
            for (int q = 0; q < 6; ++q) {
                const int i = 6 * hh + q;
                const float x1 = bk[i], x2 = bk[i + 12], c = rcL[q], sn = rcL[8 + q];
                kb[2 * q] = bf16_lo(pack_bf16(x1 * c - x2 * sn, 0.f));
                kb[2 * q + 1] = bf16_lo(pack_bf16(x2 * c + x1 * sn, 0.f));
            }
#pragma unroll
            for (int tt = 0; tt < TT; ++tt) {
                float k[12], qf[12];
#pragma unroll
                for (int c = 0; c < 3; ++c) {
                    const int ap = 3 * hd + c, ft = ap >> 2, a = ap & 3;
#pragma unroll
                    for (int b2 = 0; b2 < 4; ++b2) k[4 * c + b2] = acc[ft * TT + tt][4 * a + b2];
                }
#pragma unroll
                for (int q = 0; q < 6; ++q) {
                    const uint32_t u = (HALF || tt == 0) ? qp[tt][hd][q] : qstash[w][hd * 6 + q][lane];
                    qf[2 * q] = bf16_lo(u);
                    qf[2 * q + 1] = bf16_hi(u);
                }
                float s[5] = {0.f, 0.f, 0.f, 0.f, 0.f};
#pragma unroll
                for (int i = 0; i < 12; ++i) {
                    s[0] += qf[i] * quad_bcast<0>(k[i]);
                    s[1] += qf[i] * quad_bcast<1>(k[i]);
                    s[2] += qf[i] * quad_bcast<2>(k[i]);
                    s[3] += qf[i] * quad_bcast<3>(k[i]);
                    s[4] += qf[i] * kb[i];
                }
#pragma unroll
                for (int j = 0; j < 5; ++j) s[j] = half_sum(s[j]);
                const float m0 = quad_bcast<0>(mval[tt]), m1 = quad_bcast<1>(mval[tt]), m2 = quad_bcast<2>(mval[tt]),
                            m3 = quad_bcast<3>(mval[tt]);
                s[0] = m0 != 0.f ? s[0] : -1e30f;
                s[1] = m1 != 0.f ? s[1] : -1e30f;
                s[2] = m2 != 0.f ? s[2] : -1e30f;
                s[3] = m3 != 0.f ? s[3] : -1e30f;
                const float mx = fmaxf(fmaxf(fmaxf(s[0], s[1]), fmaxf(s[2], s[3])), s[4]);
                float den = 0.f;
#pragma unroll
                for (int j = 0; j < 5; ++j) {
                    s[j] = s[j] > -1e29f ? __builtin_amdgcn_exp2f(s[j] - mx) : 0.f;
                    den += s[j];
                }
                const float inv = 1.0f / den;
#pragma unroll
                for (int j = 0; j < 5; ++j) P[tt][hd][j] = s[j] * inv;
            }
            __builtin_amdgcn_sched_barrier(0);
        }
    }
    ATTN4_STAMP(6);
    uint32_t Pk[10];
    if constexpr (HALF) {
        const float* Pf = &P[0][0][0];
#pragma unroll
        for (int i = 0; i < 10; ++i) Pk[i] = pack_bf16(Pf[2 * i], Pf[2 * i + 1]);
    } else {
        const float* Pf = &P[0][0][0];
#pragma unroll
        for (int i = 0; i < 20; ++i) qstash[w][i][lane] = pack_bf16(Pf[2 * i], Pf[2 * i + 1]);
    }
    __builtin_amdgcn_sched_barrier(0);
    zero_acc<3 * TT>(acc);
    wave_gemm<TT, 3, 24, true, HALF ? 4 : kAttn4VPF>(panel, kRowB, t0, 0, p.wv + (size_t)(3 * w) * 24 * 64 + lane, 24 * 64, acc);
    ATTN4_STAMP(7);
    load_head_bias(p.bv, w, hh, bb);
    {
        float* Pf = &P[0][0][0];
#pragma unroll
        for (int i = 0; i < 10 * TT; ++i) {
            const uint32_t u = HALF ? Pk[i % 10] : qstash[w][i][lane];
            Pf[2 * i] = bf16_lo(u);
            Pf[2 * i + 1] = bf16_hi(u);
        }
    }
    if (PROJ) __syncthreads();
#pragma unroll
    for (int hd = 0; hd < 4; ++hd) {
        const int head = 4 * w + hd;
        float bvv[12];
#pragma unroll
        for (int i = 0; i < 12; ++i) bvv[i] = bf16_lo(pack_bf16(p.bias_v[head * kDH + 12 * hh + i], 0.f));
#pragma unroll
        for (int tt = 0; tt < TT; ++tt) {
            float v[12], o[12];
            head_values<TT>(acc, tt, hd, bb[hd], v);
#pragma unroll
            for (int i = 0; i < 12; ++i)
                o[i] = P[tt][hd][0] * quad_bcast<0>(v[i]) + P[tt][hd][1] * quad_bcast<1>(v[i]) +
                       P[tt][hd][2] * quad_bcast<2>(v[i]) + P[tt][hd][3] * quad_bcast<3>(v[i]) + P[tt][hd][4] * bvv[i];
            if (PROJ) {
                const bool ok = tok[tt] >= 0;
#pragma unroll
                for (int i = 0; i < 3; ++i)
                    *reinterpret_cast<u32x2*>(panel + panel_off((t0 + tt) * 32 + tk, head * 48 + hh * 24 + 8 * i, kRowB)) =
                        u32x2{ok ? pack_bf16(o[4 * i], o[4 * i + 1]) : 0u, ok ? pack_bf16(o[4 * i + 2], o[4 * i + 3]) : 0u};
            } else if (tok[tt] >= 0) {
                u32x2* d = reinterpret_cast<u32x2*>(p.obuf + (long)tok[tt] * kC + head * kDH + hh * 12);
                d[0] = u32x2{pack_bf16(o[0], o[1]), pack_bf16(o[2], o[3])};
                d[1] = u32x2{pack_bf16(o[4], o[5]), pack_bf16(o[6], o[7])};
                d[2] = u32x2{pack_bf16(o[8], o[9]), pack_bf16(o[10], o[11])};
            }
        }
        __builtin_amdgcn_sched_barrier(0);
    }
    if (!PROJ) return;
    __syncthreads();
    ATTN4_STAMP(8);
    zero_acc<3 * TT>(acc);
    wave_gemm<TT, 3, 24, false>(panel, kRowB, t0, 0, p.wo + (size_t)(3 * w) * 24 * 64 + lane, 24 * 64, acc);
    ATTN4_STAMP(9);
    __syncthreads();
    if constexpr (HALF) {
        float* stage = reinterpret_cast<float*>(panel) + w * (32 * 96);
        epi_stage(acc, stage);
        epi_rmw<8>(0, pr, stage, 96 * w, p.bo, p.mm, p.gate_chunk, true, p.h_rw);
    } else {
        epilogue_gate_residual_lds<3>(acc, pr, reinterpret_cast<float*>(panel) + w * (32 * 96), 96 * w, p.bo, p.mm, p.gate_chunk,
                                      true, p.h_rw);
    }
    ATTN4_STAMP(10);
    ATTN4_STAMP_FLUSH
}

template <int MAXL>
__device__ __forceinline__ void prologue_micro_attn(unsigned char* panel, const PanelRows* pr, const ProjParams& p) {
    const int L = p.ax.len;
    for (int item = threadIdx.x; item < kPanel * kH; item += 256) {
        const int row = item >> 4, head = item & 15;
        const int token = pr->tok[row];
        const int tkc = token < 0 ? 0 : token;
        const int seq = tkc / L;
        const __bf16* sbase = p.qkv_small + (long)seq * L * (3 * kC) + head * kDH;
        const u32x4* qp = reinterpret_cast<const u32x4*>(p.qkv_small + (long)tkc * (3 * kC) + head * kDH);
        u32x4 qv[3], kk[MAXL][3], vv[MAXL][3];
        float mk[MAXL];
#pragma unroll
        for (int i = 0; i < 3; ++i) qv[i] = qp[i];
#pragma unroll
        for (int j = 0; j < MAXL; ++j) {
            const int jc = j < L ? j : L - 1;
            mk[j] = p.mk.at((long)seq * L + jc);
            const u32x4* kp = reinterpret_cast<const u32x4*>(sbase + (long)jc * (3 * kC) + kC);
#pragma unroll
            for (int i = 0; i < 3; ++i) kk[j][i] = kp[i];
        }
        if (MAXL <= 4) {
#pragma unroll
            for (int j = 0; j < MAXL; ++j) {
                const int jc = j < L ? j : L - 1;
                const u32x4* vp = reinterpret_cast<const u32x4*>(sbase + (long)jc * (3 * kC) + 2 * kC);
#pragma unroll
                for (int i = 0; i < 3; ++i) vv[j][i] = vp[i];
            }
        }
        float q[24];
#pragma unroll
        for (int i = 0; i < 3; ++i)
#pragma unroll
            for (int j = 0; j < 4; ++j) {
                q[8 * i + 2 * j] = bf16_lo(qv[i][j]);
                q[8 * i + 2 * j + 1] = bf16_hi(qv[i][j]);
            }
        float s[MAXL + 1];
        float mx = -1e30f;
#pragma unroll
        for (int j = 0; j < MAXL; ++j) {
            float d = 0.f;
#pragma unroll
            for (int i = 0; i < 3; ++i)
#pragma unroll
                for (int jj = 0; jj < 4; ++jj)
                    d += q[8 * i + 2 * jj] * bf16_lo(kk[j][i][jj]) + q[8 * i + 2 * jj + 1] * bf16_hi(kk[j][i][jj]);
            s[j] = (j < L && mk[j] != 0.f) ? d : -1e30f;
            mx = fmaxf(mx, s[j]);
        }
        if (MAXL > 4) {
#pragma unroll
            for (int j = 0; j < MAXL; ++j) {
                const int jc = j < L ? j : L - 1;
                const u32x4* vp = reinterpret_cast<const u32x4*>(sbase + (long)jc * (3 * kC) + 2 * kC);
#pragma unroll
                for (int i = 0; i < 3; ++i) vv[j][i] = vp[i];
            }
        }
        {
            const float* bk = p.bias_k + head * kDH;
            const float* rc = p.rope + (long)L * kRopeRow;
            float d = 0.f;
#pragma unroll
            for (int hh = 0; hh < 2; ++hh)
#pragma unroll
                for (int pp = 0; pp < 6; ++pp) {
                    const int i = 6 * hh + pp;
                    const float x1 = bk[i], x2 = bk[i + 12], c = rc[16 * hh + pp], sn = rc[16 * hh + 8 + pp];
                    const float k1 = bf16_lo(pack_bf16(x1 * c - x2 * sn, 0.f));
                    const float k2 = bf16_lo(pack_bf16(x2 * c + x1 * sn, 0.f));
                    d += q[hh * 12 + 2 * pp] * k1 + q[hh * 12 + 2 * pp + 1] * k2;
                }
            s[MAXL] = d;
            mx = fmaxf(mx, d);
        }
        float o[24];
#pragma unroll
        for (int i = 0; i < 24; ++i) o[i] = 0.f;
        float den = 0.f;
#pragma unroll
        for (int j = 0; j < MAXL; ++j) {
            const float pj = s[j] > -1e29f ? __builtin_amdgcn_exp2f(s[j] - mx) : 0.f;
            den += pj;
#pragma unroll
            for (int i = 0; i < 3; ++i)
#pragma unroll
                for (int jj = 0; jj < 4; ++jj) {
                    o[8 * i + 2 * jj] += pj * bf16_lo(vv[j][i][jj]);
                    o[8 * i + 2 * jj + 1] += pj * bf16_hi(vv[j][i][jj]);
                }
        }
        {
            const float pj = __builtin_amdgcn_exp2f(s[MAXL] - mx);
            den += pj;
            const float* bv = p.bias_v + head * kDH;
#pragma unroll
            for (int i = 0; i < 24; ++i) o[i] += pj * bf16_lo(pack_bf16(bv[i], 0.f));
        }
        const float inv = token >= 0 ? 1.0f / den : 0.f;
#pragma unroll
        for (int i = 0; i < 3; ++i)
            *reinterpret_cast<u32x4*>(panel + panel_off(row, head * 48 + i * 16, kRowB)) =
                u32x4{pack_bf16(o[8 * i] * inv, o[8 * i + 1] * inv), pack_bf16(o[8 * i + 2] * inv, o[8 * i + 3] * inv),
                      pack_bf16(o[8 * i + 4] * inv, o[8 * i + 5] * inv), pack_bf16(o[8 * i + 6] * inv, o[8 * i + 7] * inv)};
    }
}

template <int MODE>
__global__ __launch_bounds__(256, 2) void k_proj(const ProjParams p) {
    constexpr int K = (MODE == 1) ? kIpaFeat : kC;
    constexpr int ROWB = K * 2;
    constexpr int KS = K / 16;
    __shared__ __attribute__((aligned(16))) unsigned char smem[sizeof(PanelRows) + kPanel * ROWB];
    PanelRows* pr = reinterpret_cast<PanelRows*>(smem);
    unsigned char* panel = smem + sizeof(PanelRows);
    setup_rows_linear(pr, (long)blockIdx.x * kPanel, p.nrows, p.mm);
    __syncthreads();
    if (MODE == 2) {
        if (p.ax.len <= 4) prologue_micro_attn<4>(panel, pr, p);
        else prologue_micro_attn<8>(panel, pr, p);
    } else {
        prologue_bf16<K>(panel, pr, p.a_bf16);
    }
    __syncthreads();
    const int w = __builtin_amdgcn_readfirstlane(wave_id()), lane = lane_id();
    f32x16 acc[6];
    zero_acc<6>(acc);
    wave_gemm<2, 3, KS, false>(panel, ROWB, 0, 0, p.w + (size_t)(3 * w) * KS * 64 + lane, KS * 64, acc);
    if (MODE == 1) {
        epilogue_gate_residual<2, 3>(acc, pr, 96 * w, p.bias, p.mm, p.gate_chunk, p.gated != 0, p.h);
    } else {
        __syncthreads();
        epilogue_gate_residual_lds<3>(acc, pr, reinterpret_cast<float*>(panel) + w * (32 * 96), 96 * w, p.bias, p.mm,
                                      p.gate_chunk, p.gated != 0, p.h);
    }
}
// ... 542 lines not shown
```

### mdgen_amd/csrc/k_small.hip

```cpp
#include "kernels.h"

namespace mdg {

__global__ __launch_bounds__(384) void k_temb(const float* __restrict__ t_rows, float tmul,
                                              const float* __restrict__ w0, const float* __restrict__ b0,
                                              const float* __restrict__ w2, const float* __restrict__ b2,
                                              float* __restrict__ out) {
    __shared__ float emb[256];
    __shared__ float h1[kC];
    const int r = blockIdx.x, c = threadIdx.x;
    const float t = t_rows[r] * tmul;
    if (c < 256) {
        const int i = c & 127;
        const float f = expf(-9.210340371976184f * (float)i / 128.0f);
        const float a = t * f;
        emb[c] = (c < 128) ? cosf(a) : sinf(a);
    }
    __syncthreads();
    float acc = b0[c];
    const float* wr = w0 + (long)c * 256;
    for (int i = 0; i < 256; ++i) acc += wr[i] * emb[i];
    h1[c] = acc / (1.0f + expf(-acc));
    __syncthreads();
    float acc2 = b2[c];
    const float* wr2 = w2 + (long)c * kC;
    for (int i = 0; i < kC; ++i) acc2 += wr2[i] * h1[i];
    out[(long)r * kC + c] = acc2 / (1.0f + expf(-acc2));
}

__global__ __launch_bounds__(256) void k_adaln(const float* __restrict__ st, int nrows, const float* __restrict__ w,
                                               const float* __restrict__ b, int nout, float* __restrict__ mod) {
    const int o = blockIdx.x * 4 + wave_id();
    if (o >= nout) return;
    const int lane = lane_id();
    float wv[6];
#pragma unroll
    for (int i = 0; i < 6; ++i) wv[i] = w[(long)o * kC + lane + 64 * i];
    const float bo = b[o];
    for (int r = 0; r < nrows; ++r) {
        const float* s = st + (long)r * kC;
        float a = 0.f;
#pragma unroll
        for (int i = 0; i < 6; ++i) a += wv[i] * s[lane + 64 * i];
        a = wave_sum(a);
        if (lane == 0) mod[(long)r * nout + o] = a + bo;
    }
}

__global__ void k_rope_table(float* __restrict__ rope, const float* __restrict__ inv_freq, int npos) {
    const int i = blockIdx.x * blockDim.x + threadIdx.x;
    if (i >= npos * 16) return;
    const int pos = i / 16, k = i % 16;
    const int h = k >> 3, j = k & 7;
    float c = 0.f, sn = 0.f;
    if (j < 6) {
        const float a = (float)pos * inv_freq[6 * h + j];
        c = cosf(a);
        sn = sinf(a);
    }
    rope[(long)pos * kRopeRow + h * 16 + j] = c;
    rope[(long)pos * kRopeRow + h * 16 + 8 + j] = sn;
}

__global__ void k_gather_f32(const float* __restrict__ src, const int* __restrict__ idx, float scale,
                             float* __restrict__ dst, int n) {
    const int i = blockIdx.x * blockDim.x + threadIdx.x;
    if (i < n) dst[i] = idx[i] >= 0 ? scale * src[idx[i]] : 0.f;
}

__global__ void k_pack_rows(const float* __restrict__ w, int ld, const int* __restrict__ rowmap, int nft, int ksteps,
                            float scale, bf16x8* __restrict__ dst, int kappa, int part) {
    const long i = (long)blockIdx.x * blockDim.x + threadIdx.x;
    const long total = (long)nft * ksteps * 64;
    if (i >= total) return;
    const int lane = (int)(i & 63);
    const long fk = i >> 6;
    const int ks = (int)(fk % ksteps), ft = (int)(fk / ksteps);
    const int row = rowmap[ft * 32 + (lane & 31)];
    const int hh = lane >> 5;
    bf16x8 v;
#pragma unroll
    for (int j = 0; j < 8; ++j) {
        const int k = kappa ? ks * 16 + 8 * (j >> 2) + 4 * hh + (j & 3) : ks * 16 + hh * 8 + j;
        const float x = row >= 0 && k < ld ? w[(long)row * ld + k] * scale : 0.f;
        const __bf16 hi = (__bf16)x;
        v[j] = part ? (__bf16)(x - (float)hi) : hi;
    }
    dst[i] = v;
}

constexpr int kEmbLd = 29, kEmbK = 14;
template <bool POS, bool IPA, int kEmbTok>
__global__ __launch_bounds__(256) void k_embed(const EmbedParams p) {
    __shared__ float xs[kEmbTok * kEmbLd];
    __shared__ float cs[kEmbTok * kEmbLd];
    __shared__ int ms[kEmbTok];
    __shared__ int tpos[kEmbTok];
    __shared__ int tipa[kEmbTok];
    const int tid = threadIdx.x;
    const long tok0 = (long)blockIdx.x * kEmbTok;
    if (tid < kEmbTok) {
        long t = tok0 + tid;
        t = t < p.N ? t : p.N - 1;
        const int l = (int)(t % p.L), b = (int)(t / ((long)p.T * p.L));
        ms[tid] = 0;
        tpos[tid] = l * kC;
        tipa[tid] = (b * p.L + l) * kC;
    }
    __syncthreads();
    {
        constexpr int NIT = (kEmbTok * 28 + 255) / 256;
        float a[NIT], b[NIT];
#pragma unroll
        for (int it = 0; it < NIT; ++it) {
            const int i0 = tid + 256 * it;
            const int i = i0 < kEmbTok * 28 ? i0 : kEmbTok * 28 - 1;
            const int tk = i / 28, d = i % 28;
            long t = tok0 + tk;
            t = t < p.N ? t : p.N - 1;
            const int dc = d < p.D ? d : 0;
            a[it] = p.x[t * p.D + dc];
            b[it] = p.x_cond[t * p.D + dc];
        }
#pragma unroll
        for (int it = 0; it < NIT; ++it) {
            const int i = tid + 256 * it;
            if (i >= kEmbTok * 28) break;
            const int tk = i / 28, d = i % 28;
            const bool ok = tok0 + tk < p.N && d < p.D;
            xs[tk * kEmbLd + d] = ok ? a[it] : 0.f;
            cs[tk * kEmbLd + d] = ok ? b[it] : 0.f;
            if (ok && b[it] != 0.f) atomicOr(&ms[tk], 2);
        }
    }
    const int w = __builtin_amdgcn_readfirstlane(wave_id()), lane = lane_id(), hh = lane >> 5, j = lane & 31;
    const int nk = (p.D + 1) >> 1;
    float wl[3][kEmbK], wc[3][kEmbK], b0[3], me0[3], me1[3];
#pragma unroll
    for (int ct = 0; ct < 3; ++ct) {
        const int c = 96 * w + 32 * ct + j;
#pragma unroll
        for (int ks = 0; ks < kEmbK; ++ks) {
            const int o = ((w * 3 + ct) * kEmbK + ks) * 64 + lane;
            wl[ct][ks] = p.wl_pack[o];
            wc[ct][ks] = p.wc_pack[o];
        }
        b0[ct] = p.bl[c] + p.bc[c];
        me0[ct] = p.mask_emb[c];
        me1[ct] = p.mask_emb[kC + c];
    }
    __syncthreads();
    if (tid < kEmbTok) {
        const long t = tok0 + tid;
        if (t < p.N && p.x_cond_mask[t]) ms[tid] |= 1;
    }
    __syncthreads();
#pragma unroll 1
    for (int rt = 0; rt < kEmbTok / 32; ++rt) {
        if (tok0 + rt * 32 >= p.N) break;
        f32x16 acc[3];
#pragma unroll
        for (int ct = 0; ct < 3; ++ct)
#pragma unroll
            for (int r = 0; r < 16; ++r) acc[ct][r] = 0.f;
        const float* xr = xs + (rt * 32 + j) * kEmbLd + hh;
#pragma unroll
        for (int ks = 0; ks < kEmbK; ++ks) {
            if (ks < nk) {
                const float a = xr[2 * ks];
#pragma unroll
                for (int ct = 0; ct < 3; ++ct) acc[ct] = __builtin_amdgcn_mfma_f32_32x32x2f32(a, wl[ct][ks], acc[ct], 0, 0, 0);
            }
        }
        if (__builtin_amdgcn_ballot_w64((ms[rt * 32 + j] & 2) != 0) != 0) {
            const float* cr = cs + (rt * 32 + j) * kEmbLd + hh;
#pragma unroll
            for (int ks = 0; ks < kEmbK; ++ks) {
                if (ks < nk) {
                    const float a = cr[2 * ks];
#pragma unroll
                    for (int ct = 0; ct < 3; ++ct) acc[ct] = __builtin_amdgcn_mfma_f32_32x32x2f32(a, wc[ct][ks], acc[ct], 0, 0, 0);
                }
            }
        }
#pragma unroll
        for (int r0 = 0; r0 < 16; r0 += 4) {
            float add[4][3];
            int mrow[4];
#pragma unroll
            for (int u = 0; u < 4; ++u) {
                const int tk = rt * 32 + mfma_row(r0 + u, hh);
                mrow[u] = ms[tk];
                const int op = tpos[tk], oi = tipa[tk];
#pragma unroll
                for (int ct = 0; ct < 3; ++ct) {
                    const int c = 96 * w + 32 * ct + j;
                    float v = 0.f;
                    if (POS) v += p.pos_embed[op + c];
                    if (IPA) v += p.ipa_out[oi + c];
                    add[u][ct] = v;
                }
            }
#pragma unroll
            for (int u = 0; u < 4; ++u) {
                const long t = tok0 + rt * 32 + mfma_row(r0 + u, hh);
                if (t < p.N) {
#pragma unroll
                    for (int ct = 0; ct < 3; ++ct)
                        p.h[t * kC + 96 * w + 32 * ct + j] = acc[ct][r0 + u] + b0[ct] + ((mrow[u] & 1) ? me1[ct] : me0[ct]) + add[u][ct];
                }
            }
        }
    }
}
// ... 220 lines not shown
            }
            const float mj = sm[jj];
            const float l = dot + hwh * d2 + 1e5f * (mi * mj - 1.0f);
            lg[jj] = mj < 0.f ? -3.0e38f : l;
            tmax = fmaxf(tmax, lg[jj]);
        }
        const float mnew = fmaxf(mrun, tmax);
        const float alpha = expf(mrun - mnew);
        mrun = mnew;
        den *= alpha;
#pragma unroll
        for (int c = 0; c < 32; ++c) o[c] *= alpha;
#pragma unroll
        for (int pt = 0; pt < 8; ++pt) {
            op[pt][0] *= alpha; op[pt][1] *= alpha; op[pt][2] *= alpha;
        }
#pragma unroll
        for (int jj = 0; jj < kIpaKT; ++jj) {
            const float pw = lg[jj] > -1.0e38f ? expf(lg[jj] - mnew) : 0.f;
            den += pw;
#pragma unroll
            for (int c = 0; c < 32; c += 4) {
                const f32x4 vv = *reinterpret_cast<const f32x4*>(&sv[jj][c]);
                o[c] += pw * vv[0]; o[c + 1] += pw * vv[1]; o[c + 2] += pw * vv[2]; o[c + 3] += pw * vv[3];
            }
#pragma unroll
            for (int pt = 0; pt < 8; ++pt) {
                op[pt][0] += pw * svp[jj][3 * pt];
                op[pt][1] += pw * svp[jj][3 * pt + 1];
                op[pt][2] += pw * svp[jj][3 * pt + 2];
            }
        }
    }
    if (!qok) return;
    if (nsl > 1) {
        float* rec = p.part + (((long)sl * p.ngroups * p.L + gi) * 4 + hd) * kIpaFwdRec;
        rec[0] = mrun;
        rec[1] = den;
#pragma unroll
        for (int c = 0; c < 32; ++c) rec[2 + c] = o[c];
#pragma unroll
        for (int pt = 0; pt < 8; ++pt)
#pragma unroll
            for (int x = 0; x < 3; ++x) rec[34 + 3 * pt + x] = op[pt][x];
        return;
    }
    const float inv = 1.0f / den;
    if (p.stats) p.stats[gi * 4 + hd] = mrun + logf(den);
    ipa_store_features(p, gi, hd, o, op, inv, Ri, ti);
}

__global__ __launch_bounds__(256) void k_ipa_attn_merge(const IpaAttnParams p) {
    const long idx = (long)blockIdx.x * blockDim.x + threadIdx.x;
    const long mtot = (long)p.ngroups * p.L;
    if (idx >= mtot * 4) return;
    const int hd = (int)(idx & 3);
    const long gi = idx >> 2;
    const int i = (int)(gi % p.L);
    const int b = (int)((gi / p.L) % p.B);
    float Ri[9], ti[3];
#pragma unroll
    for (int k = 0; k < 9; ++k) Ri[k] = p.rot[((long)b * p.L + i) * 9 + k];
#pragma unroll
    for (int k = 0; k < 3; ++k) ti[k] = p.trans[((long)b * p.L + i) * 3 + k];
    float m = -3.0e38f;
    for (int z = 0; z < p.nsplit; ++z) m = fmaxf(m, p.part[(((long)z * mtot + gi) * 4 + hd) * kIpaFwdRec]);
    float o[32], op[8][3], den = 0.f;
#pragma unroll
    for (int c = 0; c < 32; ++c) o[c] = 0.f;
#pragma unroll
    for (int pt = 0; pt < 8; ++pt) op[pt][0] = op[pt][1] = op[pt][2] = 0.f;
    for (int z = 0; z < p.nsplit; ++z) {
        const float* rec = p.part + (((long)z * mtot + gi) * 4 + hd) * kIpaFwdRec;
        const float a = expf(rec[0] - m);
        den += a * rec[1];
#pragma unroll
        for (int c = 0; c < 32; ++c) o[c] += a * rec[2 + c];
#pragma unroll
        for (int pt = 0; pt < 8; ++pt)
#pragma unroll
            for (int x = 0; x < 3; ++x) op[pt][x] += a * rec[34 + 3 * pt + x];
    }
    const float inv = 1.0f / den;
    if (p.stats) p.stats[gi * 4 + hd] = m + logf(den);
    ipa_store_features(p, gi, hd, o, op, inv, Ri, ti);
}

__global__ void k_path_plan(const float* __restrict__ t, const float* __restrict__ x0, const float* __restrict__ x1,
                            float* __restrict__ xt, float* __restrict__ ut, long per_sample, long total, int gvp) {
    const long i = (long)blockIdx.x * blockDim.x + threadIdx.x;
    if (i >= total) return;
    const float tb = t[i / per_sample];
    float a, sg, da, ds;
    if (gvp) {
        const float hp = 1.57079632679489662f;
        const float sn = sinf(tb * hp), cs = cosf(tb * hp);
        a = sn; sg = cs; da = hp * cs; ds = -hp * sn;
    } else {
        a = tb; sg = 1.0f - tb; da = 1.0f; ds = -1.0f;
    }
    const float v1 = x1[i], v0 = x0[i];
    xt[i] = a * v1 + sg * v0;
    ut[i] = da * v1 + ds * v0;
}

__global__ __launch_bounds__(256) void k_masked_mse(const float* __restrict__ pred, const float* __restrict__ target,
                                                    const float* __restrict__ mask, float* __restrict__ loss,
                                                    long per_sample) {
    __shared__ float red[2][4];
    const long base = (long)blockIdx.x * per_sample;
    float num = 0.f, den = 0.f;
    long i = threadIdx.x;
    for (; i + 7 * 256 < per_sample; i += 8 * 256) {
        float pv[8], tv[8], mv[8];
#pragma unroll
        for (int u = 0; u < 8; ++u) {
            pv[u] = pred[base + i + 256 * u];
            tv[u] = target[base + i + 256 * u];
            mv[u] = mask[base + i + 256 * u];
        }
#pragma unroll
        for (int u = 0; u < 8; ++u) {
            const float d = pv[u] - tv[u];
            num += d * d * mv[u];
            den += mv[u];
        }
    }
    for (; i < per_sample; i += 256) {
        const float d = pred[base + i] - target[base + i], m = mask[base + i];
        num += d * d * m;
        den += m;
    }
    num = wave_sum(num);
    den = wave_sum(den);
    if (lane_id() == 0) {
        red[0][wave_id()] = num;
        red[1][wave_id()] = den;
    }
    __syncthreads();
    if (threadIdx.x == 0)
        loss[blockIdx.x] = (red[0][0] + red[0][1] + red[0][2] + red[0][3]) / (red[1][0] + red[1][1] + red[1][2] + red[1][3]);
}

void launch_temb(const float* t_rows, int nrows, float tmul, const float* w0, const float* b0, const float* w2,
                 const float* b2, float* silu_out, hipStream_t s) {
    hipLaunchKernelGGL(k_temb, dim3(nrows), dim3(384), 0, s, t_rows, tmul, w0, b0, w2, b2, silu_out);
}
void launch_adaln(const float* st, int nrows, const float* w, const float* b, int nout, float* mod, hipStream_t s) {
    hipLaunchKernelGGL(k_adaln, dim3((nout + 3) / 4), dim3(256), 0, s, st, nrows, w, b, nout, mod);
}
void launch_rope_table(float* rope, const float* inv_freq, int npos, hipStream_t s) {
    hipLaunchKernelGGL(k_rope_table, dim3((npos * 16 + 255) / 256), dim3(256), 0, s, rope, inv_freq, npos);
}
void launch_gather_f32(const float* src, const int* idx, float scale, float* dst, int n, hipStream_t s) {
    hipLaunchKernelGGL(k_gather_f32, dim3((n + 255) / 256), dim3(256), 0, s, src, idx, scale, dst, n);
}
void launch_pack_rows(const float* w, int ld, const int* rowmap, int nft, int ksteps, float scale, bf16x8* dst,
                      hipStream_t s, int kappa, int part) {
    const long total = (long)nft * ksteps * 64;
    hipLaunchKernelGGL(k_pack_rows, dim3((unsigned)((total + 255) / 256)), dim3(256), 0, s, w, ld, rowmap, nft, ksteps,
                       scale, dst, kappa, part);
}
void launch_path_plan(const float* t, const float* x0, const float* x1, float* xt, float* ut, long per_sample, long B,
                      int gvp, hipStream_t s) {
    const long total = per_sample * B;
    hipLaunchKernelGGL(k_path_plan, dim3((unsigned)((total + 255) / 256)), dim3(256), 0, s, t, x0, x1, xt, ut, per_sample,
                       total, gvp);
}
constexpr int kMseChunk = 8192;
__global__ __launch_bounds__(256) void k_masked_mse_partial(const float* __restrict__ pred, const float* __restrict__ target,
                                                            const float* __restrict__ mask, long per_sample, int nchunk,
                                                            float* __restrict__ part) {
    __shared__ float red[2][4];
    const long b = blockIdx.y;
    const long lo = (long)blockIdx.x * kMseChunk, hi = lo + kMseChunk < per_sample ? lo + kMseChunk : per_sample;
    const long base = b * per_sample;
    float num = 0.f, den = 0.f;
#pragma unroll 8
    for (long i = lo + threadIdx.x; i < hi; i += 256) {
        const float m = mask[base + i];
        den += m;
        if (pred) {
            const float d = pred[base + i] - target[base + i];
            num += d * d * m;
        }
    }
    num = wave_sum(num);
    den = wave_sum(den);
    if (lane_id() == 0) {
        red[0][wave_id()] = num;
        red[1][wave_id()] = den;
    }
    __syncthreads();
    if (threadIdx.x == 0) {
        float* o = part + (b * nchunk + blockIdx.x) * 2;
        o[0] = (red[0][0] + red[0][1]) + (red[0][2] + red[0][3]);
        o[1] = (red[1][0] + red[1][1]) + (red[1][2] + red[1][3]);
    }
}
__global__ __launch_bounds__(64) void k_masked_mse_final(const float* __restrict__ part, int nchunk, float* __restrict__ loss,
                                                         float* __restrict__ den_out) {
    const float* p = part + (long)blockIdx.x * nchunk * 2;
    float num = 0.f, den = 0.f;
    for (int i = threadIdx.x; i < nchunk; i += 64) {
        num += p[2 * i];
        den += p[2 * i + 1];
    }
    num = wave_sum(num);
    den = wave_sum(den);
    if (threadIdx.x == 0) {
        if (loss) loss[blockIdx.x] = num / den;
        if (den_out) den_out[blockIdx.x] = den;
    }
}
void launch_masked_mse(const float* pred, const float* target, const float* mask, float* loss, long per_sample, long B,
                       hipStream_t s, float* scratch, size_t scratch_floats, float* den_out) {
    const long nchunk = (per_sample + kMseChunk - 1) / kMseChunk;
    if (scratch && nchunk > 1 && (size_t)(2 * B * nchunk) <= scratch_floats) {
        hipLaunchKernelGGL(k_masked_mse_partial, dim3((unsigned)nchunk, (unsigned)B), dim3(256), 0, s, pred, target, mask, per_sample,
                           (int)nchunk, scratch);
        hipLaunchKernelGGL(k_masked_mse_final, dim3((unsigned)B), dim3(64), 0, s, scratch, (int)nchunk, loss, den_out);
        return;
    }
    hipLaunchKernelGGL(k_masked_mse, dim3((unsigned)B), dim3(256), 0, s, pred, target, mask, loss, per_sample);
}
__global__ void k_pack_embed(const float* __restrict__ w, int D, float* __restrict__ pack) {
    const int lane = threadIdx.x, blk = blockIdx.x;
    const int ks = blk % kEmbK, tile = blk / kEmbK;
    const int c = 32 * tile + (lane & 31), d = 2 * ks + (lane >> 5);
    pack[blk * 64 + lane] = d < D ? w[(long)c * D + d] : 0.f;
}
void launch_pack_embed(const float* w, int D, float* pack, hipStream_t s) {
    hipLaunchKernelGGL(k_pack_embed, dim3(4 * 3 * kEmbK), dim3(64), 0, s, w, D, pack);
}
void launch_embed(const EmbedParams& p, hipStream_t s) {
    const dim3 b(256);
    if ((p.N + 127) / 128 >= 384) {
        const dim3 g((unsigned)((p.N + 127) / 128));
        if (p.pos_embed && p.ipa_out) hipLaunchKernelGGL((k_embed<true, true, 128>), g, b, 0, s, p);
        else if (p.pos_embed) hipLaunchKernelGGL((k_embed<true, false, 128>), g, b, 0, s, p);
        else if (p.ipa_out) hipLaunchKernelGGL((k_embed<false, true, 128>), g, b, 0, s, p);
        else hipLaunchKernelGGL((k_embed<false, false, 128>), g, b, 0, s, p);
    } else {
        const dim3 g((unsigned)((p.N + 31) / 32));
        if (p.pos_embed && p.ipa_out) hipLaunchKernelGGL((k_embed<true, true, 32>), g, b, 0, s, p);
        else if (p.pos_embed) hipLaunchKernelGGL((k_embed<true, false, 32>), g, b, 0, s, p);
        else if (p.ipa_out) hipLaunchKernelGGL((k_embed<false, true, 32>), g, b, 0, s, p);
        else hipLaunchKernelGGL((k_embed<false, false, 32>), g, b, 0, s, p);
    }
}
void launch_ipa_init(const float* aa_emb, const int64_t* aatype, const float* rel7, const float* w7, const float* b7,
                     float* h, int ngroups, int B, int L, hipStream_t s) {
    hipLaunchKernelGGL(k_ipa_init, dim3((unsigned)((long)ngroups * L)), dim3(384), 0, s, aa_emb, aatype, rel7, w7, b7, h,
                       B, L);
}
void launch_write_floats(const float* host_vals, int n, float* dst, hipStream_t s) {
    for (int o = 0; o < n; o += 128) {
        FloatChunk c;
        c.n = n - o < 128 ? n - o : 128;
        for (int i = 0; i < c.n; ++i) c.v[i] = host_vals[o + i];
        hipLaunchKernelGGL(k_write_floats, dim3(1), dim3(128), 0, s, c, dst + o);
    }
}
void launch_add_inplace(float* dst, const float* src, long n, hipStream_t s) {
    hipLaunchKernelGGL(k_add_inplace, dim3((unsigned)((n + 255) / 256)), dim3(256), 0, s, dst, src, n);
}
void launch_ipa_attn(const IpaAttnParams& p, hipStream_t s) {
    if (p.L >= 24) {
        const int nqt = (p.L + 255) / 256;
        const long nblk = (long)p.ngroups * 4 * nqt, mtot = (long)p.ngroups * p.L;
        IpaAttnParams q = p;
        int nsplit = p.part ? (int)((64 + nblk - 1) / nblk) : 1;
        const int ntile = (p.L + kIpaKT - 1) / kIpaKT;
        if (nsplit > ntile) nsplit = ntile;
        if (nsplit > 16) nsplit = 16;
        while (nsplit > 1 && (size_t)nsplit * mtot * 4 * kIpaFwdRec > p.part_floats) --nsplit;
        q.nsplit = nsplit;
        hipLaunchKernelGGL(k_ipa_attn_tiled, dim3((unsigned)nblk, (unsigned)nsplit), dim3(256), 0, s, q);
        if (nsplit > 1) hipLaunchKernelGGL(k_ipa_attn_merge, dim3((unsigned)((mtot * 4 + 255) / 256)), dim3(256), 0, s, q);
        return;
    }
    const long total = (long)p.ngroups * p.L * 4;
    hipLaunchKernelGGL(k_ipa_attn, dim3((unsigned)((total + 255) / 256)), dim3(256), 0, s, p);
}

}
```

### mdgen_amd/csrc/kernels.h

```cpp
#pragma once
#include "common.h"

namespace mdg {

struct QkvParams {
    const float* h;
    long nrows;
    AxisMap ax;
    ModMap mm;
    int shift_chunk, scale_chunk;
    const bf16x8 *wq, *wk, *wv;
    const float *bq, *bk, *bv;
    const float* rope;
    unsigned char *qf, *kf, *vf;
    __bf16* qkv_small;
    int panels_per_seq;
    uint32_t* vmask;
    int vmask_stride;
    const float *bias_k, *bias_v;
    MaskMap mk;
    __bf16* obuf;
    float* h_rw;
    const bf16x8* wo;
    const float* bo;
    int gate_chunk;
};

struct ProjParams {
    float* h;
    long nrows;
    ModMap mm;
    int gate_chunk;
    int gated;
    const bf16x8* w;
    const float* bias;
    const __bf16* a_bf16;
    const __bf16* qkv_small;
    AxisMap ax;
    MaskMap mk;
    const float *bias_k, *bias_v;
    const float* rope;
};

struct MlpParams {
    float* h;
    long nrows;
    ModMap mm;
    int shift_chunk, scale_chunk, gate_chunk;
    const bf16x8 *w1, *w2;
    const float *b1, *b2;
    unsigned long long* trace;
    long trace_cap;
    const __bf16* o;
    const bf16x8* wo;
    const float* bo;
    int gate_chunk_o;
    float* part;
    float* hupd;
    unsigned* counters;
};
constexpr int kMlpSplit = 3;
constexpr int kMlpSplitMaxPanels = 96;

struct MlpRowsParams {
    float* h;
    long nrows;
    ModMap mm;
    int shift_chunk, scale_chunk, gate_chunk;
    const unsigned char* wstream;
    const float *b1, *b2;
    unsigned long long* trace;
    long trace_cap;
    const float* b2g;
    const bf16x8* tail_w;
    const float* tail_b;
    const float* tail_mod;
    int tail_D, tail_euler;
    float tail_dt;
    float* tail_x;
    float* tail_out;
    const float *emb_base, *emb_mdelta, *emb_xcond;
    const bf16x8 *emb_wl_hi, *emb_wl_lo, *emb_wc_hi, *emb_wc_lo;
    const int64_t* emb_cmask;
    int emb_T, emb_L;
};
void launch_sub_f32(const float* a, const float* b, float* dst, int n, hipStream_t s);
void launch_embed_base(const float* bl, const float* bc, const float* mask_emb, const float* pos_embed, const float* ipa_out, int S,
                       int BL, int L, float* base, hipStream_t s);

struct LnLinearParams {
    const float* h;
    long nrows;
    ModMap mm;
    const bf16x8* w;
    const float* bias;
    float* out;
    int nout;
};

struct FinalParams {
    const float* h;
    long nrows;
    ModMap mm;
    int shift_chunk, scale_chunk;
    const bf16x8* w;
    const float* bias;
    int D;
    int euler;
    float dt;
    float* x;
    float* out;
};

static_assert((kFragBytes - kFragV) * kH >= 4 * 64 + 4 * 1 + 256,
              "the key-validity words (<= ntile + 64 of them per sequence, 256-byte aligned) must fit the slack the V^T fragments leave");
__host__ __device__ inline int flash_vmask_stride(int ntile) { return (ntile + 64) & ~63; }
__host__ __device__ inline size_t flash_vmask_offset(long nseq, int ntile) {
    return (((size_t)nseq * kH * ntile * kFragV) + 255) & ~(size_t)255;
}

struct FlashParams {
    AxisMap ax;
    MaskMap mk;
    const unsigned char *qf, *kf, *vf;
    const float *bias_k, *bias_v;
    const float* rope;
    __bf16* obuf;
    const uint32_t* vmask;
    int vmask_stride;
    int force_robust;
    int rotate;
};

struct FlashProjParams {
    FlashParams f;
    float* h;
    ModMap mm;
    int gate_chunk;
    const bf16x8* wo;
    const float* bo;
};

struct EmbedParams {
    const float *x, *x_cond;
    const int64_t* x_cond_mask;
    const float *wl, *bl, *wc, *bc;
    const float *wl_pack, *wc_pack;
    const float* mask_emb;
    const float* pos_embed;
    const float* ipa_out;
    float* h;
    long N;
    int T, L, D;
};

struct IpaAttnParams {
    const float* proj;
    const float *rot, *trans;
    const float* mask_bl;
    const float* head_w;
    __bf16* feat;
    float* feat32;
    float* stats;
    int ngroups, B, L;
    int nsplit;
    float* part;
    size_t part_floats;
};
constexpr int kIpaFwdRec = 58;

struct FloatChunk {
    float v[128];
// ... 78 lines not shown
};
inline bool linear_streams(LinearForm f) { return f == LinearForm::StreamF32Rows || f == LinearForm::StreamBf16Rows; }
inline bool dw_wide(DwForm f) { return f >= DwForm::Wide && f <= DwForm::WideXbfDYbf; }
inline bool dw_x_bf16(DwForm f) { return f == DwForm::WideXbf || f == DwForm::WideXbfDYbf; }
inline bool dw_dy_bf16(DwForm f) { return f == DwForm::WideDYbf || f == DwForm::WideXbfDYbf; }
inline bool attn_seq(TrainAttnForm f) { return f == TrainAttnForm::Seq || f == TrainAttnForm::SeqRope; }

struct LinShape { long n; int m, k, lda, ldw, wtrans; bool a_al, w_al, a_bf16; };
inline bool linear_vec(const LinShape& q) {
    return !q.wtrans && q.k % 64 == 0 && (q.lda & (q.a_bf16 ? 7 : 3)) == 0 && (q.ldw & 3) == 0 && q.a_al && q.w_al;
}
inline LinearForm linear_form(bool bf16, const LinShape& q, bool stream) {
    if (!bf16) return LinearForm::F32;
    if (!linear_vec(q)) return LinearForm::Plain;
    if (stream && q.n >= 1024 && q.m % 384 == 0) return q.a_bf16 ? LinearForm::StreamBf16Rows : LinearForm::StreamF32Rows;
    if (q.n >= 1024 && q.m > 128) return LinearForm::Wide;
    return q.n <= 2048 ? LinearForm::Small : LinearForm::Fast;
}

struct DwShape { long n; int m, k, ldy, ldx; bool al; };
inline bool dw_vec(const DwShape& q) { return ((q.ldy | q.m | q.ldx | q.k) & 7) == 0 && q.al; }
inline int dw_nsplit(long n, int m, int k, size_t part_floats) {
    const int tiles = ((m + 127) / 128) * ((k + 127) / 128);
    int nsplit = (int)((n + 511) / 512);
    const int want = (512 + tiles - 1) / tiles;
    if (nsplit > want) nsplit = want;
    if (nsplit > 128) nsplit = 128;
    if (nsplit < 1) nsplit = 1;
    while (nsplit > 1 && (size_t)nsplit * m * (k + 1) > part_floats) --nsplit;
    return nsplit;
}
inline DwForm dw_form(bool bf16, const DwShape& q, size_t part_floats, bool x_bf16, bool dy_bf16) {
    if (!bf16) return DwForm::F32;
    if (!dw_vec(q)) return DwForm::Plain;
    if (q.n >= 4096 && (size_t)q.m * (q.k + 1) <= part_floats)
        return x_bf16 ? (dy_bf16 ? DwForm::WideXbfDYbf : DwForm::WideXbf) : (dy_bf16 ? DwForm::WideDYbf : DwForm::Wide);
    return DwForm::Fast;
}
inline bool dw_bias_rides(DwForm f, const DwShape& q, size_t part_floats) {
    return dw_wide(f) || (f == DwForm::Fast && (size_t)dw_nsplit(q.n, q.m, q.k, part_floats) * q.m * (q.k + 1) <= part_floats);
}

inline bool slice_plan(long nrows, long tokens_per_group, int ncols, size_t part_floats, long* ng, int* rps, int* spg) {
    *ng = (nrows + tokens_per_group - 1) / tokens_per_group;
    *rps = 64;
    while (*rps > 4 && *ng * ((tokens_per_group + *rps - 1) / *rps) < 256) *rps /= 2;
    *spg = (int)((tokens_per_group + *rps - 1) / *rps);
    while ((size_t)*ng * *spg * ncols > part_floats && *rps < (1 << 24)) {
        *rps *= 2;
        *spg = (int)((tokens_per_group + *rps - 1) / *rps);
    }
    return (size_t)*ng * *spg * ncols <= part_floats;
}
inline bool slices_fit(long nrows, long tokens_per_group, int ncols, size_t part_floats) {
    long ng; int rps, spg;
    return slice_plan(nrows, tokens_per_group, ncols, part_floats, &ng, &rps, &spg);
}
inline GateBwdForm gate_bwd_form(long nrows, long tokens_per_group, size_t part_floats) {
    return slices_fit(nrows, tokens_per_group, kC, part_floats) ? GateBwdForm::Sums : GateBwdForm::MulColsum;
}
inline LnBwdForm ln_bwd_form(long nrows, long tokens_per_group, size_t part_floats, bool adjacent) {
    return adjacent && slices_fit(nrows, tokens_per_group, 2 * kC, part_floats) ? LnBwdForm::Sums : LnBwdForm::ColsumsLnBwd;
}
bool attn16_seq_form(const AxisMap& ax);
inline TrainAttnForm train_attn_form(bool bf16, const AxisMap& ax) {
    return !bf16 ? TrainAttnForm::Exact : attn16_seq_form(ax) ? TrainAttnForm::SeqRope : TrainAttnForm::Chunked;
}

void launch32_ln_mod(const float* x, long nrows, const ModMap& mm, int shift_chunk, int scale_chunk, int affine, float eps,
                     float* y, hipStream_t s, float* keep, bool y_bf16);
struct LinearParams;
void launch32_linear(const LinearParams& p, hipStream_t s);
void launch_linear(const LinearParams& p, LinearForm form, hipStream_t s);
void launch16_pack_wstream(const float* const* src, int nsrc, int seg, int ld, int m, int k, int turned, void* out, hipStream_t s);
struct DwParams {
    const float* dy; int ldy;
    const float* x; int ldx;
    long n; int mseg, nseg, k;
    float* dw[3];
    float* db[3];
    float* part; size_t part_floats;
};
inline DwShape dw_shape(const DwParams& p) {
    return DwShape{p.n, p.mseg * p.nseg, p.k, p.ldy, p.ldx, (((unsigned long long)p.dy | (unsigned long long)p.x) & 15) == 0};
}
void launch_dw(const DwParams& p, DwForm form, hipStream_t s);
void launch32_colsum(const float* a, int lda, const float* b, int ldb, const float* roww, int mode, long nrows, int ncols,
                     long tokens_per_group, float eps, float* out, long ldo, float* part, size_t part_floats, hipStream_t s);
void launch32_ln_bwd(const float* x, const float* dy, long nrows, const ModMap& mm, int scale_chunk, int affine, float eps,
                     float* dx, int accumulate, hipStream_t s);
void launch32_gate_mul(const float* a, long nrows, const ModMap& mm, int gate_chunk, int gated, float* out, hipStream_t s);
void launch32_attn_bwd(const float* qkv, int ld, const AxisMap& ax, const MaskMap& mk, const float* bias_k,
                       const float* bias_v, const float* inv_freq, const float* o, const float* dout, float* dqkv,
                       float* stats, float* dbias, hipStream_t s, const float* lse_in);
void launch32_rope_bwd(float* buf, long ntok, int ld, long pos_div, int pos_mod, const float* inv_freq, float qscale,
                       hipStream_t s);
void launch32_loss_grad(const float* pred, const float* target, const float* mask, long per_sample, long B, float* den,
                        float* dpred, hipStream_t s, float* scratch, size_t scratch_floats);
void launch32_sum_frames(const float* a, int B, int T, int L, float* out, hipStream_t s);
void launch32_ipa_bwd(const IpaAttnParams& f, const float* dfeat, float* dproj, float* dhw, float* qrec, float* dheadw,
                      hipStream_t s, float* part, size_t part_floats);
void launch32_gated_add(float* h, const float* u, long nrows, const ModMap& mm, int gate_chunk, int gated, hipStream_t s);
void launch32_gated_sum(float* h, const float* x, const float* u, long nrows, const ModMap& mm, int gate_chunk, hipStream_t s);
void launch32_gate_ln_mod(const float* xp, const float* up, long nrows, const ModMap& gm, int gate_chunk, const ModMap& mm,
                          int shift_chunk, int scale_chunk, float eps, float* y, float* keep, hipStream_t s, bool y_bf16);
void launch32_indicator(const int64_t* cm, long n, float* ind0, float* ind1, hipStream_t s);
void launch32_embed_rows_bwd(const float* dx0, const int64_t* aatype, int ngroups, int B, int L, float* dw, hipStream_t s);
void launch32_temb_bwd(const float* t_rows, int nrows, float tmul, const float* w0, const float* b0, const float* w2,
                       const float* b2, const float* dst, float* emb, float* h1, float* dpre1, float* dpre2, hipStream_t s);
void launch32_rope(float* buf, long ntok, int ld, long pos_div, int pos_mod, const float* inv_freq, hipStream_t s);
bool launch32_skinny_wt(const float* x, int ldx, const float* W, int ldw, int nb, int m, long K, float* out, float* part,
                        size_t part_floats, hipStream_t s);
struct GateBwdParams {
    const float *dh, *u;
    long nrows; ModMap mm; int gate_chunk;
    float* du; bool du_bf16;
    long tokens_per_group; float* out; long ldo;
    float* part; size_t part_floats;
};
void launch32_gate_bwd(const GateBwdParams& p, GateBwdForm form, hipStream_t s);
struct LnBwdParams {
    const float *x, *dy;
    long nrows; ModMap mm; int scale_chunk; float eps;
    float* dx; int accumulate;
    long tokens_per_group; float *dshift, *dscale; long ldo;
    float* part; size_t part_floats;
};
void launch32_ln_mod_bwd(const LnBwdParams& p, LnBwdForm form, hipStream_t s);
void launch32_transpose(const float* src, int rows, int cols, float* dst, hipStream_t s, int ldd);
struct TrainAttnParams {
    const float* qkv; int ld;
    AxisMap ax; MaskMap mk;
    const float *bias_k, *bias_v, *inv_freq;
    float *out, *lse;
    const float* dout;
    float *dqkv, *stats, *dbias;
    bool dqkv_bf16;
};
void launch_train_attn(const TrainAttnParams& p, TrainAttnForm form, hipStream_t s);
void launch_train_attn_bwd(const TrainAttnParams& p, TrainAttnForm form, hipStream_t s);
void launch32_attn(const float* qkv, int ld, const AxisMap& ax, const MaskMap& mk, const float* bias_k, const float* bias_v,
                   const float* inv_freq, float* out, hipStream_t s, float* lse_out);

void launch_sumsq(const float* g, long n, float scale, float* partial, int nblocks, float* out, hipStream_t s);
void launch_adam(float* p, const float* g, float* m, float* v, long n, float lr, float beta1, float beta2, float eps,
                 float weight_decay, int adamw, float bc1, float bc2_sqrt, float grad_scale, const float* sumsq,
                 float max_norm, hipStream_t s);
void launch_ema(float* ema, const float* p, long n, float one_minus_decay, hipStream_t s);

void launch_temb(const float* t_rows, int nrows, float tmul, const float* w0, const float* b0, const float* w2,
                 const float* b2, float* silu_out, hipStream_t s);
void launch_adaln(const float* st, int nrows, const float* w, const float* b, int nout, float* mod, hipStream_t s);
void launch_rope_table(float* rope, const float* inv_freq, int npos, hipStream_t s);
void launch_gather_f32(const float* src, const int* idx, float scale, float* dst, int n, hipStream_t s);
void launch_pack_rows(const float* w, int ld, const int* rowmap, int nft, int ksteps, float scale, bf16x8* dst,
                      hipStream_t s, int kappa = 0, int part = 0);
void launch_ipa_init(const float* aa_emb, const int64_t* aatype, const float* rel7, const float* w7, const float* b7,
                     float* h, int ngroups, int B, int L, hipStream_t s);
void launch_add_inplace(float* dst, const float* src, long n, hipStream_t s);
void launch_write_floats(const float* host_vals, int n, float* dst, hipStream_t s);
void launch_rel7(const float* r1, const float* t1, const float* r2, const float* t2, float* out7, long n, hipStream_t s);

constexpr int kOdeMaxTerms = 7;
constexpr int kOdeMaxParts = 1024;
struct OdeTerms {
    const float* k[kOdeMaxTerms];
    float c[kOdeMaxTerms];
    int nk;
};
struct OdeNorm {
    const float *a, *b;
    const float* k[kOdeMaxTerms];
    float e[kOdeMaxTerms];
    double atol, rtol;
    int mode;
};
void launch_ode_combine(float* out, const float* y0, const OdeTerms& p, long n, hipStream_t s);
int ode_norm_parts(long n);
void launch_ode_norm(const OdeNorm& p, long n, double* part, double* out, hipStream_t s);
void launch_ode_dense(float* out, const float* y0, const float* y1, const float* f0, const float* f1, const float* ym, float dt,
                      float sfrac, long n, hipStream_t s);

void launch_rigid_compose(long n, const float* r1, const float* t1, const float* r2, const float* t2, float* ro,
                          float* to, hipStream_t s);
void launch_rigid_invert(long n, const float* r, const float* t, float* ro, float* to, hipStream_t s);
void launch_rigid_apply(long n, long ppf, const float* r, const float* t, const float* pts, float* out, int inverse,
                        hipStream_t s);
void launch_quat_to_rot(long n, const float* q, int normalize, float* rot, hipStream_t s);
void launch_from_3_points(long n, const float* pnx, const float* org, const float* pxy, float* rot, float* trans,
                          hipStream_t s);
void launch_rot_to_quat(long n, const float* rot, float* q, hipStream_t s);
void launch_prep_latents(int B, int T, int L, int tps, int bcast, int cond_interval, const float* rots, const float* trans,
                         const float* tors, float* latents, float* x_cond, int64_t* x_cond_mask, hipStream_t s);
void launch_samples_to_atom14(int B, int T, int L, int D, int tps, const float* samples, const float* rot0,
                              const float* trans0, const int64_t* seqres, const float* default_frames,
                              const float* lit_positions, const int64_t* atom14_group, const float* atom14_mask,
                              float* atom14, int out_T, int out_t0, hipStream_t s);
void launch_atom14_to_cond(int B, int L, const float* atom14, long in_bstride, const int64_t* seqres,
                           const int64_t* a37to14, const float* a37mask, const int64_t* chi_idx, const float* chi_mask,
                           float* rots, float* trans, float* tors, float* tmask, hipStream_t s);

}
```

### mdgen_amd/csrc/panel.h

```cpp
#pragma once
#include "common.h"

namespace mdg {

__device__ __forceinline__ void lds_barrier() { asm volatile("s_waitcnt lgkmcnt(0)\n\ts_barrier" ::: "memory"); }

__device__ __forceinline__ int panel_off(int row, int byte_in_row, int rowb) {
    return row * rowb + (byte_in_row ^ ((row & 15) << 4));
}

__device__ __forceinline__ bf16x8 panel_frag(const unsigned char* panel, const int rowb, int tile, int ks) {
    const int lane = lane_id();
    const int row = tile * 32 + (lane & 31);
    return *reinterpret_cast<const bf16x8*>(panel + panel_off(row, ks * 32 + (lane >> 5) * 16, rowb));
}

template <int TT, int FT, int KSTEPS, bool TRANS, int PF = 4>
__device__ __forceinline__ void wave_gemm(const unsigned char* panel, const int rowb, const int tile0, const int ks0,
                                          const bf16x8* __restrict__ wfrag, const int wtile_stride,
                                          f32x16* acc) {
    static_assert(PF < KSTEPS, "prefetch depth");
    bf16x8 wring[PF + 1][FT];
    bf16x8 aring[2][TT];
#pragma unroll
    for (int p = 0; p < PF; ++p)
#pragma unroll
        for (int f = 0; f < FT; ++f) wring[p][f] = wfrag[(size_t)f * wtile_stride + p * 64];
#pragma unroll
    for (int t = 0; t < TT; ++t) aring[0][t] = panel_frag(panel, rowb, tile0 + t, ks0);
    __builtin_amdgcn_sched_barrier(0);
#pragma unroll
    for (int ks = 0; ks < KSTEPS; ++ks) {
        if (ks + PF < KSTEPS) {
#pragma unroll
            for (int f = 0; f < FT; ++f)
                wring[(ks + PF) % (PF + 1)][f] = wfrag[(size_t)f * wtile_stride + (ks + PF) * 64];
        }
        if (ks + 1 < KSTEPS) {
#pragma unroll
            for (int t = 0; t < TT; ++t) aring[(ks + 1) & 1][t] = panel_frag(panel, rowb, tile0 + t, ks0 + ks + 1);
        }
        __builtin_amdgcn_sched_barrier(0);
#pragma unroll
        for (int t = 0; t < TT; ++t)
#pragma unroll
            for (int f = 0; f < FT; ++f) {
                if (TRANS)
                    acc[f * TT + t] = __builtin_amdgcn_mfma_f32_32x32x16_bf16(wring[ks % (PF + 1)][f], aring[ks & 1][t],
                                                                             acc[f * TT + t], 0, 0, 0);
                else
                    acc[t * FT + f] = __builtin_amdgcn_mfma_f32_32x32x16_bf16(aring[ks & 1][t], wring[ks % (PF + 1)][f],
                                                                             acc[t * FT + f], 0, 0, 0);
            }
        __builtin_amdgcn_sched_barrier(0);
    }
}

template <int N>
__device__ __forceinline__ void zero_acc(f32x16* acc) {
#pragma unroll
    for (int i = 0; i < N; ++i)
#pragma unroll
        for (int r = 0; r < 16; ++r) acc[i][r] = opaque_zero();
}

struct PanelRows {
    int tok[kPanel];
    int moff[kPanel];
    int uniform;
    int pad_[3];
};

__device__ __forceinline__ void set_uniform(PanelRows* pr, int tid, long t, long mo) {
    const int mo0 = __builtin_amdgcn_readfirstlane((int)mo);
    const int t0 = __builtin_amdgcn_readfirstlane((int)t);
    const bool same = t < 0 || (int)mo == mo0;
    const bool all = __builtin_amdgcn_ballot_w64(same) == ~0ull;
    if (tid == 0) pr->uniform = (t0 >= 0 && all) ? mo0 : -1;
}

__device__ __forceinline__ void setup_rows_axis(PanelRows* pr, const AxisMap ax, int seq, int pos0, const ModMap mm, int nrows = kPanel) {
    if (threadIdx.x < kPanel) {
        const int pos = pos0 + threadIdx.x;
        long t = -1, mo = 0;
        if (pos < ax.len && (int)threadIdx.x < nrows) {
            t = ax.token(seq, pos);
            mo = mm.row_off(t);
        }
        pr->tok[threadIdx.x] = (int)t;
        pr->moff[threadIdx.x] = (int)mo;
        set_uniform(pr, threadIdx.x, t, mo);
    }
}

__device__ __forceinline__ void setup_rows_linear(PanelRows* pr, long row0, long nrows, const ModMap mm,
                                                  int tid = threadIdx.x) {
    if (tid >= 0 && tid < kPanel) {
        long t = row0 + tid, mo = 0;
        if (t < nrows) mo = mm.row_off(t); else t = -1;
        pr->tok[tid] = (int)t;
        pr->moff[tid] = (int)mo;
        set_uniform(pr, tid, t, mo);
    }
}

template <bool AFFINE, int B0, int B1, bool UNI>
__device__ __forceinline__ void prologue_ln_impl(unsigned char* panel, const PanelRows* pr, const float* __restrict__ x,
                                            const ModMap mm, int shift_chunk, int scale_chunk, float eps,
                                            const int w, const int lane, const int um) {
    constexpr int ROWB = kC * 2;
    constexpr int RB = 4, NB = kPanel / (4 * RB);
    static_assert(0 <= B0 && B0 < B1 && B1 <= NB, "batch range");
    int t[NB][RB];
    f32x2 v[NB][RB][3];
    f32x2 scu[3], shu[3];
    if (UNI) {
        const unsigned char* mb = reinterpret_cast<const unsigned char*>(mm.mod);
        const unsigned osh = ((unsigned)um + (unsigned)(shift_chunk * kC)) * 4u + (unsigned)lane * 8u;
        const unsigned osc = ((unsigned)um + (unsigned)(scale_chunk * kC)) * 4u + (unsigned)lane * 8u;
#pragma unroll
        for (int i = 0; i < 3; ++i) {
            scu[i] = *reinterpret_cast<const f32x2*>(mb + osc + 512u * i);
            shu[i] = *reinterpret_cast<const f32x2*>(mb + osh + 512u * i);
        }
    }
#pragma unroll
    for (int b = B0; b < B1; ++b) {
        const int r0 = 4 * RB * b + RB * w;
#pragma unroll
        for (int j = 0; j < RB; ++j) {
            t[b][j] = pr->tok[r0 + j];
            const unsigned off = (unsigned)(t[b][j] < 0 ? 0 : t[b][j]) * (unsigned)(kC * 4) + (unsigned)lane * 8u;
            const unsigned char* xb = reinterpret_cast<const unsigned char*>(x);
#pragma unroll
            for (int i = 0; i < 3; ++i) v[b][j][i] = *reinterpret_cast<const f32x2*>(xb + off + 512u * i);
        }
        f32x2 sc[RB][3], sh[RB][3];
#pragma unroll
        for (int j = 0; j < RB; ++j) {
            if (UNI) {
#pragma unroll
                for (int i = 0; i < 3; ++i) {
                    sc[j][i] = scu[i];
                    sh[j][i] = shu[i];
                }
            } else {
                const unsigned mo = AFFINE ? 0u : (unsigned)pr->moff[r0 + j];
                const unsigned char* mb = reinterpret_cast<const unsigned char*>(mm.mod);
                const unsigned osh = (mo + (unsigned)(shift_chunk * kC)) * 4u + (unsigned)lane * 8u;
                const unsigned osc = (mo + (unsigned)(scale_chunk * kC)) * 4u + (unsigned)lane * 8u;
#pragma unroll
                for (int i = 0; i < 3; ++i) {
                    sc[j][i] = *reinterpret_cast<const f32x2*>(mb + osc + 512u * i);
                    sh[j][i] = *reinterpret_cast<const f32x2*>(mb + osh + 512u * i);
                }
            }
        }
        float mean[RB], rstd[RB];
#pragma unroll
        for (int j = 0; j < RB; ++j) {
            const float s = (v[b][j][0][0] + v[b][j][0][1]) + (v[b][j][1][0] + v[b][j][1][1]) + (v[b][j][2][0] + v[b][j][2][1]);
            mean[j] = wave_sum(s) * (1.0f / kC);
        }
#pragma unroll
        for (int j = 0; j < RB; ++j) {
            float q = 0.f;
#pragma unroll
            for (int i = 0; i < 3; ++i) {
                v[b][j][i][0] -= mean[j];
                v[b][j][i][1] -= mean[j];
                q += v[b][j][i][0] * v[b][j][i][0] + v[b][j][i][1] * v[b][j][i][1];
            }
            rstd[j] = 1.0f / sqrtf(wave_sum(q) * (1.0f / kC) + eps);
        }
#pragma unroll
        for (int j = 0; j < RB; ++j) {
#pragma unroll
            for (int i = 0; i < 3; ++i) {
                const float m0 = AFFINE ? sc[j][i][0] : 1.0f + sc[j][i][0];
                const float m1 = AFFINE ? sc[j][i][1] : 1.0f + sc[j][i][1];
                const float y0 = v[b][j][i][0] * rstd[j] * m0 + sh[j][i][0];
                const float y1 = v[b][j][i][1] * rstd[j] * m1 + sh[j][i][1];
                *reinterpret_cast<uint32_t*>(panel + panel_off(r0 + j, 4 * lane + 256 * i, ROWB)) =
                    t[b][j] >= 0 ? pack_bf16(y0, y1) : 0u;
            }
        }
    }
}

template <bool AFFINE, int B0 = 0, int B1 = 4>
__device__ __forceinline__ void prologue_ln(unsigned char* panel, const PanelRows* pr, const float* __restrict__ x,
                                            const ModMap mm, int shift_chunk, int scale_chunk, float eps,
                                            const int w = wave_id(), const int lane = lane_id()) {
    const int um = AFFINE ? 0 : pr->uniform;
    if (um >= 0) prologue_ln_impl<AFFINE, B0, B1, true>(panel, pr, x, mm, shift_chunk, scale_chunk, eps, w, lane, um);
    else prologue_ln_impl<AFFINE, B0, B1, false>(panel, pr, x, mm, shift_chunk, scale_chunk, eps, w, lane, 0);
}

template <int K>
__device__ __forceinline__ void prologue_bf16(unsigned char* panel, const PanelRows* pr, const __bf16* __restrict__ src) {
    constexpr int ROWB = K * 2;
    constexpr int CPR = ROWB / 16;
    constexpr int NIT = kPanel * CPR / 256;
    static_assert(kPanel * CPR % 256 == 0, "whole iterations");
    u32x4 v[NIT];
    int tk[NIT];
// ... 181 lines not shown
```

Before: 127,100.

## Stage bias/rope in LDS, precompute l4 bias table, use DPP fmac and zero-C MFMA

Several independent changes. The QKV and attention kernels now stage the per-projection biases and the RoPE rows into LDS at kernel start, and the epilogues read from there instead of global memory. A bias table for the L=4 attention (rotated bias_k and packed bias_v) is precomputed at finalize. The quad-broadcast multiply-adds become inline v_fmac_f32_dpp/v_mul_f32_dpp. wave_gemm can start its first MFMA from a zero C operand instead of calling zero_acc separately. The cost is more LDS per block, which may lower occupancy, plus hand-written DPP asm that needs fence nops.

Result: faster. 130,400, median of 6 (+2.6%).

```diff
diff --git a/mdgen_amd/csrc/api.hip b/mdgen_amd/csrc/api.hip
--- a/mdgen_amd/csrc/api.hip
+++ b/mdgen_amd/csrc/api.hip
@@ -61,6 +61,7 @@
     bf16x8 *wq = nullptr, *wk = nullptr, *wv_flash = nullptr, *wv_small = nullptr, *wo = nullptr;
     float *bq = nullptr, *bk = nullptr, *bv_flash = nullptr, *bv_small = nullptr, *bo = nullptr;
     float *bias_k = nullptr, *bias_v = nullptr;
+    uint32_t* l4tab = nullptr;
     struct { Lin q, k, v, o; int bias_k = -1, bias_v = -1; } slot;
 };
 struct FfnW {
@@ -306,6 +307,7 @@
     if (int r = c->dalloc(&m->wo, kPackCC)) return r;
     for (float** p : {&m->bq, &m->bk, &m->bv_flash, &m->bv_small, &m->bo, &m->bias_k, &m->bias_v})
         if (int r = c->dalloc(p, (size_t)kC)) return r;
+    if (int r = c->dalloc(&m->l4tab, (size_t)2 * kL4Tab)) return r;
     m->slot.q.w = SETTER(pre + "q_proj.weight", {
         WANT(kC, kC);
         launch_pack_rows(data, kC, c->map_qk, 12, kKS, qscale, m->wq, s);
@@ -611,6 +613,10 @@
         if (!w.provided) return fail(-5, "weight '%s' was not provided", w.name.c_str());
     if (!c->inv_freq_set) return fail(-5, "rot_emb.inv_freq was not provided");
     launch_rope_table(c->rope, c->inv_freq, kMaxPos + 1, (hipStream_t)stream);
+    LAUNCHCHK();
+    auto l4tab = [&](const MhaW& m) { launch_l4_bias_table(m.bias_k, m.bias_v, c->rope, m.l4tab, (hipStream_t)stream); };
+    for (const TrunkW& t : c->trunk) l4tab(t.mha_l);
+    for (const IpaW& w : c->ipa) l4tab(w.mha_l);
     LAUNCHCHK();
     c->finalized = true;
     return 0;
@@ -1149,6 +1155,7 @@
         q.bv = m.bv_small;
         q.bias_k = m.bias_k;
         q.bias_v = m.bias_v;
+        q.l4tab = m.l4tab;
         q.mk = mk;
         q.obuf = r.obufp;
         if (pl.proj == ProjAt::Attention) {
diff --git a/mdgen_amd/csrc/k_gemm.hip b/mdgen_amd/csrc/k_gemm.hip
--- a/mdgen_amd/csrc/k_gemm.hip
+++ b/mdgen_amd/csrc/k_gemm.hip
@@ -6,9 +6,80 @@
 constexpr int kRowB = kC * 2;
 constexpr int kPanelBytes = kPanel * kRowB;
 
-template <bool ROPE, int TT = 2>
+constexpr int kRopeLds = kRopeRow + 4;
+constexpr int kBiasUnits = 3 * kC / 4;
+struct QkvStage {
+    float bias[3][kC];
+    float rope[kPanel][kRopeLds];
+};
+struct Attn4Stage {
+    float bias[3][kC];
+    uint32_t tab[2][kL4Tab];
+    float rope[4][kRopeLds];
+};
+__device__ __forceinline__ const f32x4* stage_bias_src(const QkvParams& p, int u) {
+    const float* b = u < kC / 4 ? p.bq : u < 2 * (kC / 4) ? p.bk : p.bv;
+    return reinterpret_cast<const f32x4*>(b) + (u % (kC / 4));
+}
+template <int NT>
+struct QkvStager {
+    static constexpr int kUnits = kBiasUnits + kPanel * 8, kPer = (kUnits + NT - 1) / NT;
+    f32x4 r[kPer];
+    __device__ __forceinline__ void load(const QkvParams& p, int pos0, int len, int tid) {
+#pragma unroll
+        for (int i = 0; i < kPer; ++i) {
+            int u = tid + i * NT;
+            if (u >= kUnits) u = kUnits - 1;
+            const int v = u >= kBiasUnits ? u - kBiasUnits : 0;
+            int pos = pos0 + (v >> 3);
+            if (pos > len) pos = len;
+            const f32x4* rs = reinterpret_cast<const f32x4*>(p.rope + (long)pos * kRopeRow) + (v & 7);
+            r[i] = *(u < kBiasUnits ? stage_bias_src(p, u) : rs);
+        }
+    }
+    __device__ __forceinline__ void store(QkvStage* st, int tid) const {
+#pragma unroll
+        for (int i = 0; i < kPer; ++i) {
+            const int u = tid + i * NT;
+            if (u < kBiasUnits) {
+                reinterpret_cast<f32x4*>(&st->bias[0][0])[u] = r[i];
+            } else if (u < kUnits) {
+                const int v = u - kBiasUnits;
+                *reinterpret_cast<f32x4*>(&st->rope[v >> 3][4 * (v & 7)]) = r[i];
+            }
+        }
+    }
+};
+struct Attn4Stager {
+    static constexpr int kTab0 = kBiasUnits, kRope0 = kTab0 + 2 * kL4Tab / 4, kUnits = kRope0 + 4 * 8;
+    static_assert(kUnits <= 512 && kBiasUnits > 256, "two units per thread, the first always a bias unit");
+    f32x4 r[2];
+    __device__ __forceinline__ void load(const QkvParams& p, int tid) {
+        r[0] = *stage_bias_src(p, tid);
+        int u = tid + 256;
+        if (u >= kUnits) u = kUnits - 1;
+        const f32x4* src = u < kTab0    ? stage_bias_src(p, u < kTab0 ? u : 0)
+                           : u < kRope0 ? reinterpret_cast<const f32x4*>(p.l4tab) + (u - kTab0)
+                                        : reinterpret_cast<const f32x4*>(p.rope) + (u - kRope0);
+        r[1] = *src;
+    }
+    __device__ __forceinline__ void store(Attn4Stage* st, int tid) const {
+        reinterpret_cast<f32x4*>(&st->bias[0][0])[tid] = r[0];
+        const int u = tid + 256;
+        if (u < kTab0) {
+            reinterpret_cast<f32x4*>(&st->bias[0][0])[u] = r[1];
+        } else if (u < kRope0) {
+            reinterpret_cast<f32x4*>(&st->tab[0][0])[u - kTab0] = r[1];
+        } else if (u < kUnits) {
+            const int v = u - kRope0;
+            *reinterpret_cast<f32x4*>(&st->rope[v >> 3][4 * (v & 7)]) = r[1];
+        }
+    }
+};
+
+template <bool ROPE, int TT = 2, bool STAGED = false>
 __device__ __forceinline__ void epilogue_heads_T(const f32x16* acc , const PanelRows* pr, int w,
-                                                 const float* __restrict__ bias_perm, const float* __restrict__ rope,
+                                                 const float* bias_perm, const float* rope,
                                                  bool small, int pos0, int len, int seq, int ntile, int tile0,
                                                  unsigned char* __restrict__ frag, __bf16* __restrict__ small_dst,
                                                  int which) {
@@ -31,7 +102,7 @@
         if (pos > len) pos = len;
         posv[tt] = pos;
         if (ROPE) {
-            const f32x4* rc = reinterpret_cast<const f32x4*>(rope + (long)pos * kRopeRow + 16 * hh);
+            const f32x4* rc = reinterpret_cast<const f32x4*>(STAGED ? rope + row * kRopeLds + 16 * hh : rope + (long)pos * kRopeRow + 16 * hh);
 #pragma unroll
             for (int i = 0; i < 4; ++i) rq[tt][i] = rc[i];
         }
@@ -94,7 +165,7 @@
 
 template <int TT = 2>
 __device__ __forceinline__ void epilogue_v_flash(const f32x16* acc , int w,
-                                                 const float* __restrict__ bias_perm, int seq, int ntile, int tile0,
+                                                 const float* bias_perm, int seq, int ntile, int tile0,
                                                  unsigned char* __restrict__ vf) {
     const int lane = lane_id(), hh = lane >> 5, n = lane & 31;
 #pragma unroll
@@ -212,6 +283,9 @@
 template <bool SMALL, bool PRE = false>
 __global__ __launch_bounds__(256, 2) void k_ln_qkv(const QkvParams p) {
     __shared__ __attribute__((aligned(16))) unsigned char smem[sizeof(PanelRows) + kPanelBytes];
+    __shared__ __attribute__((aligned(16))) unsigned char stage_[SMALL ? 16 : sizeof(QkvStage)];
+    QkvStage* const stage = reinterpret_cast<QkvStage*>(stage_);
+    QkvStager<256> stager;
     PanelRows* pr = reinterpret_cast<PanelRows*>(smem);
     unsigned char* panel = smem + sizeof(PanelRows);
     int seq = 0, pos0 = 0, tile0 = 0;
@@ -222,6 +296,7 @@
         const int pn = blockIdx.x - seq * p.panels_per_seq;
         pos0 = pn * kPanel;
         tile0 = pn * 2;
+        stager.load(p, pos0, p.ax.len, threadIdx.x);
         setup_rows_axis(pr, p.ax, seq, pos0, p.mm);
         if (wave_id() == 0) {
             const int lane = lane_id(), len = p.ax.len, pos = pos0 + lane;
@@ -238,13 +313,15 @@
     }
     QKV_STAMP(0);
     __syncthreads();
+    if (!SMALL) stager.store(stage, threadIdx.x);
     const int w = __builtin_amdgcn_readfirstlane(wave_id()), lane = lane_id();
+    const float *sbq = SMALL ? p.bq : stage->bias[0], *sbk = SMALL ? p.bk : stage->bias[1], *sbv = SMALL ? p.bv : stage->bias[2];
+    const float* srope = SMALL ? p.rope : &stage->rope[0][0];
     f32x16 acc[6];
     if (PRE) {
         prologue_bf16<kC>(panel, pr, p.obuf);
         __syncthreads();
-        zero_acc<6>(acc);
-        wave_gemm<2, 3, 24, false>(panel, kRowB, 0, 0, p.wo + (size_t)(3 * w) * 24 * 64 + lane, 24 * 64, acc);
+        wave_gemm<2, 3, 24, false, 4, true>(panel, kRowB, 0, 0, p.wo + (size_t)(3 * w) * 24 * 64 + lane, 24 * 64, acc);
         __syncthreads();
         epilogue_gate_residual_lds<3>(acc, pr, reinterpret_cast<float*>(panel) + w * (32 * 96), 96 * w, p.bo, p.mm, p.gate_chunk,
                                       true, p.h_rw);
@@ -255,26 +332,23 @@
     QKV_STAMP(1);
     const int ntile = p.ax.ntile();
     const int len = p.ax.len;
-    zero_acc<6>(acc);
-    wave_gemm<2, 3, 24, true>(panel, kRowB, 0, 0, p.wq + (size_t)(3 * w) * 24 * 64 + lane, 24 * 64, acc);
+    wave_gemm<2, 3, 24, true, 4, true>(panel, kRowB, 0, 0, p.wq + (size_t)(3 * w) * 24 * 64 + lane, 24 * 64, acc);
     QKV_STAMP(2);
-    epilogue_heads_T<true>(acc, pr, w, p.bq, p.rope, SMALL, pos0, len, seq, ntile, tile0, p.qf, p.qkv_small, 0);
+    epilogue_heads_T<true, 2, !SMALL>(acc, pr, w, sbq, srope, SMALL, pos0, len, seq, ntile, tile0, p.qf, p.qkv_small, 0);
     __builtin_amdgcn_sched_barrier(0);
     QKV_STAMP(3);
-    zero_acc<6>(acc);
-    wave_gemm<2, 3, 24, true>(panel, kRowB, 0, 0, p.wk + (size_t)(3 * w) * 24 * 64 + lane, 24 * 64, acc);
+    wave_gemm<2, 3, 24, true, 4, true>(panel, kRowB, 0, 0, p.wk + (size_t)(3 * w) * 24 * 64 + lane, 24 * 64, acc);
     QKV_STAMP(4);
-    epilogue_heads_T<true>(acc, pr, w, p.bk, p.rope, SMALL, pos0, len, seq, ntile, tile0, p.kf, p.qkv_small, 1);
+    epilogue_heads_T<true, 2, !SMALL>(acc, pr, w, sbk, srope, SMALL, pos0, len, seq, ntile, tile0, p.kf, p.qkv_small, 1);
     __builtin_amdgcn_sched_barrier(0);
     QKV_STAMP(5);
-    zero_acc<6>(acc);
     if (SMALL) {
-        wave_gemm<2, 3, 24, true>(panel, kRowB, 0, 0, p.wv + (size_t)(3 * w) * 24 * 64 + lane, 24 * 64, acc);
+        wave_gemm<2, 3, 24, true, 4, true>(panel, kRowB, 0, 0, p.wv + (size_t)(3 * w) * 24 * 64 + lane, 24 * 64, acc);
         epilogue_heads_T<false>(acc, pr, w, p.bv, nullptr, true, pos0, len, seq, ntile, tile0, nullptr, p.qkv_small, 2);
     } else {
-        wave_gemm<2, 3, 24, false>(panel, kRowB, 0, 0, p.wv + (size_t)(3 * w) * 24 * 64 + lane, 24 * 64, acc);
+        wave_gemm<2, 3, 24, false, 4, true>(panel, kRowB, 0, 0, p.wv + (size_t)(3 * w) * 24 * 64 + lane, 24 * 64, acc);
         QKV_STAMP(6);
-        epilogue_v_flash(acc, w, p.bv, seq, ntile, tile0, p.vf);
+        epilogue_v_flash(acc, w, sbv, seq, ntile, tile0, p.vf);
         if ((int)blockIdx.x - seq * p.panels_per_seq == p.panels_per_seq - 1) {
             __builtin_amdgcn_sched_barrier(0);
             write_bias_slots(p, seq, w);
@@ -287,6 +361,22 @@
 __device__ __forceinline__ float quad_bcast(float v) {
     return __builtin_bit_cast(float, __builtin_amdgcn_update_dpp(0, __builtin_bit_cast(int, v), J * 0x55, 0xf, 0xf, true));
 }
+template <int J>
+__device__ __forceinline__ float fmac_dpp(float acc, float k, float q) {
+    asm("v_fmac_f32_dpp %0, %1, %2 quad_perm:[%3,%3,%3,%3] row_mask:0xf bank_mask:0xf bound_ctrl:1" : "+v"(acc) : "v"(k), "v"(q), "n"(J));
+    return acc;
+}
+template <int J>
+__device__ __forceinline__ float mul_dpp(float k, float q) {
+    float r;
+    asm("v_mul_f32_dpp %0, %1, %2 quad_perm:[%3,%3,%3,%3] row_mask:0xf bank_mask:0xf bound_ctrl:1" : "=v"(r) : "v"(k), "v"(q), "n"(J));
+    return r;
+}
+__device__ __forceinline__ void dpp_fence(float (&k)[12]) {
+    asm volatile("s_nop 1"
+                 : "+v"(k[0]), "+v"(k[1]), "+v"(k[2]), "+v"(k[3]), "+v"(k[4]), "+v"(k[5]), "+v"(k[6]), "+v"(k[7]), "+v"(k[8]), "+v"(k[9]),
+                   "+v"(k[10]), "+v"(k[11]));
+}
 __device__ __forceinline__ float half_sum(float x) {
     const auto r = __builtin_amdgcn_permlane32_swap(__float_as_uint(x), __float_as_uint(x), false, false);
     return __uint_as_float(r[0]) + __uint_as_float(r[1]);
@@ -298,6 +388,18 @@
         const int ap = 3 * hd + c, ft = ap >> 2, a = ap & 3;
 #pragma unroll
         for (int b = 0; b < 4; ++b) e[4 * c + b] = acc[ft * TT + tt][4 * a + b] + bq[c][b];
+    }
+}
+template <bool X1S>
+__device__ __forceinline__ void rotate_pair(float x1, float x2, float c, float sn, float& e0, float& e1) {
+    const float a = x2 * sn;
+    e0 = __builtin_fmaf(x1, c, -a);
+    if (X1S) {
+        const float b = x1 * sn;
+        e1 = __builtin_fmaf(x2, c, b);
+    } else {
+        const float b = x2 * c;
+        e1 = __builtin_fmaf(x1, sn, b);
     }
 }
 __device__ __forceinline__ void load_head_bias(const float* bias_perm, int w, int hh, f32x4 (&bq)[4][3]) {
@@ -314,12 +416,15 @@
     static_assert(!HALF || SPLIT, "32-row workgroups exist in the split form only");
     constexpr int TT = HALF ? 1 : 2, kRows = 32 * TT;
     __shared__ __attribute__((aligned(16))) unsigned char smem[sizeof(PanelRows) + kPanelBytes];
+    __shared__ __attribute__((aligned(16))) QkvStage stage;
+    QkvStager<512> stager;
     PanelRows* pr = reinterpret_cast<PanelRows*>(smem);
     unsigned char* panel = smem + sizeof(PanelRows);
     const int blk = SPLIT ? blockIdx.x >> 1 : blockIdx.x, half = SPLIT ? blockIdx.x & 1 : 0;
     const int seq = blk / p.panels_per_seq;
     const int pn = blk - seq * p.panels_per_seq;
     const int pos0 = pn * kRows, tile0 = pn * TT;
+    stager.load(p, pos0, p.ax.len, threadIdx.x);
     setup_rows_axis(pr, p.ax, seq, pos0, p.mm, kRows);
     if (wave_id() == 0 && half == 0) {
         const int lane = lane_id(), len = p.ax.len, pos = pos0 + lane;
@@ -334,6 +439,7 @@
         }
     }
     __syncthreads();
+    stager.store(&stage, threadIdx.x);
     const int w8 = __builtin_amdgcn_readfirstlane(wave_id()), g = w8 >> 2, w = w8 & 3, lane = lane_id();
     if (HALF) {
         if (g == 0) prologue_ln<false, 0, 1>(panel, pr, p.h, p.mm, p.shift_chunk, p.scale_chunk, 1e-6f, w, lane);
@@ -349,24 +455,21 @@
     const bool do_q = SPLIT ? half == 0 && g == 0 : g == 0, do_k = SPLIT ? half == 0 && g == 1 : g == 0;
     const bool do_v = SPLIT ? half == 1 && g == 0 : g == 1;
     if (do_q) {
-        zero_acc<3 * TT>(acc);
-        wave_gemm<TT, 3, 24, true>(panel, kRowB, 0, 0, p.wq + (size_t)(3 * w) * 24 * 64 + lane, 24 * 64, acc);
-        epilogue_heads_T<true, TT>(acc, pr, w, p.bq, p.rope, false, pos0, len, seq, ntile, tile0, p.qf, p.qkv_small, 0);
+        wave_gemm<TT, 3, 24, true, 4, true>(panel, kRowB, 0, 0, p.wq + (size_t)(3 * w) * 24 * 64 + lane, 24 * 64, acc);
+        epilogue_heads_T<true, TT, true>(acc, pr, w, stage.bias[0], &stage.rope[0][0], false, pos0, len, seq, ntile, tile0, p.qf, p.qkv_small, 0);
         __builtin_amdgcn_sched_barrier(0);
     }
     if (do_k) {
-        zero_acc<3 * TT>(acc);
-        wave_gemm<TT, 3, 24, true>(panel, kRowB, 0, 0, p.wk + (size_t)(3 * w) * 24 * 64 + lane, 24 * 64, acc);
-        epilogue_heads_T<true, TT>(acc, pr, w, p.bk, p.rope, false, pos0, len, seq, ntile, tile0, p.kf, p.qkv_small, 1);
+        wave_gemm<TT, 3, 24, true, 4, true>(panel, kRowB, 0, 0, p.wk + (size_t)(3 * w) * 24 * 64 + lane, 24 * 64, acc);
+        epilogue_heads_T<true, TT, true>(acc, pr, w, stage.bias[1], &stage.rope[0][0], false, pos0, len, seq, ntile, tile0, p.kf, p.qkv_small, 1);
         if (last) {
             __builtin_amdgcn_sched_barrier(0);
             write_bias_slots(p, seq, w, true, false, TT);
         }
     }
     if (do_v) {
-        zero_acc<3 * TT>(acc);
-        wave_gemm<TT, 3, 24, false>(panel, kRowB, 0, 0, p.wv + (size_t)(3 * w) * 24 * 64 + lane, 24 * 64, acc);
-        epilogue_v_flash<TT>(acc, w, p.bv, seq, ntile, tile0, p.vf);
+        wave_gemm<TT, 3, 24, false, 4, true>(panel, kRowB, 0, 0, p.wv + (size_t)(3 * w) * 24 * 64 + lane, 24 * 64, acc);
+        epilogue_v_flash<TT>(acc, w, stage.bias[2], seq, ntile, tile0, p.vf);
         if (last) {
             __builtin_amdgcn_sched_barrier(0);
             write_bias_slots(p, seq, w, false, true, TT);
@@ -381,15 +484,19 @@
     constexpr int TT = HALF ? 1 : 2, kRows = HALF ? 32 : kPanel;
     __shared__ __attribute__((aligned(16))) unsigned char smem[sizeof(PanelRows) + kPanelBytes];
     __shared__ uint32_t qstash[HALF ? 1 : 4][24][64];
+    __shared__ __attribute__((aligned(16))) Attn4Stage stage;
+    Attn4Stager stager;
     PanelRows* pr = reinterpret_cast<PanelRows*>(smem);
     unsigned char* panel = smem + sizeof(PanelRows);
     ATTN4_STAMP_DECL;
     ATTN4_STAMP(0);
+    stager.load(p, threadIdx.x);
     {
         const long row0 = (long)blockIdx.x * kRows, rend = row0 + kRows;
         setup_rows_linear(pr, row0, rend < p.nrows ? rend : p.nrows, p.mm);
     }
     __syncthreads();
+    stager.store(&stage, threadIdx.x);
     const int w = __builtin_amdgcn_readfirstlane(wave_id());
     constexpr int t0 = 0;
     if (HALF) prologue_ln<false, 0, 2>(panel, pr, p.h, p.mm, p.shift_chunk, p.scale_chunk, 1e-6f, w, lane_id());
@@ -409,7 +516,7 @@
 #pragma unroll
         for (int tt = 0; tt < TT; ++tt) {
             const int tc = tok[tt] < 0 ? 0 : tok[tt];
-            const f32x4* rc = reinterpret_cast<const f32x4*>(p.rope + (long)(tc & (L - 1)) * kRopeRow + 16 * hh);
+            const f32x4* rc = reinterpret_cast<const f32x4*>(&stage.rope[tc & (L - 1)][16 * hh]);
 #pragma unroll
             for (int i = 0; i < 4; ++i) rq[tt][i] = rc[i];
         }
@@ -417,10 +524,9 @@
     f32x16 acc[3 * TT];
     f32x4 bb[4][3];
     f32x4 rq[TT][4];
-    zero_acc<3 * TT>(acc);
-    wave_gemm<TT, 3, 24, true>(panel, kRowB, t0, 0, p.wq + (size_t)(3 * w) * 24 * 64 + lane, 24 * 64, acc);
+    wave_gemm<TT, 3, 24, true, 4, true>(panel, kRowB, t0, 0, p.wq + (size_t)(3 * w) * 24 * 64 + lane, 24 * 64, acc);
     ATTN4_STAMP(2);
-    load_head_bias(p.bq, w, hh, bb);
+    load_head_bias(stage.bias[0], w, hh, bb);
     load_rope(rq);
     uint32_t qp[TT][4][6];
 #pragma unroll
@@ -432,8 +538,9 @@
 #pragma unroll
             for (int q = 0; q < 6; ++q) {
                 const float c = rq[tt][q >> 2][q & 3], sn = rq[tt][2 + (q >> 2)][q & 3];
-                const float x1 = e[2 * q], x2 = e[2 * q + 1];
-                qp[tt][hd][q] = pack_bf16(x1 * c - x2 * sn, x2 * c + x1 * sn);
+                float r0, r1;
+                rotate_pair<HALF>(e[2 * q], e[2 * q + 1], c, sn, r0, r1);
+                qp[tt][hd][q] = pack_bf16(r0, r1);
             }
         }
     if constexpr (!HALF) {
@@ -444,10 +551,9 @@
     }
     ATTN4_STAMP(3);
     __builtin_amdgcn_sched_barrier(0);
-    zero_acc<3 * TT>(acc);
-    wave_gemm<TT, 3, 24, true, HALF ? 4 : kAttn4KPF>(panel, kRowB, t0, 0, p.wk + (size_t)(3 * w) * 24 * 64 + lane, 24 * 64, acc);
+    wave_gemm<TT, 3, 24, true, HALF ? 4 : kAttn4KPF, true>(panel, kRowB, t0, 0, p.wk + (size_t)(3 * w) * 24 * 64 + lane, 24 * 64, acc);
     ATTN4_STAMP(4);
-    load_head_bias(p.bk, w, hh, bb);
+    load_head_bias(stage.bias[1], w, hh, bb);
     load_rope(rq);
 #pragma unroll
     for (int tt = 0; tt < TT; ++tt)
@@ -462,9 +568,10 @@
                 for (int b2 = 0; b2 < 2; ++b2) {
                     const int q = 2 * c + b2;
                     const float cs = rq[tt][q >> 2][q & 3], sn = rq[tt][2 + (q >> 2)][q & 3];
-                    const float x1 = k[2 * q], x2 = k[2 * q + 1];
-                    acc[ft * TT + tt][4 * a + 2 * b2] = x1 * cs - x2 * sn;
-                    acc[ft * TT + tt][4 * a + 2 * b2 + 1] = x2 * cs + x1 * sn;
+                    float r0, r1;
+                    rotate_pair<HALF>(k[2 * q], k[2 * q + 1], cs, sn, r0, r1);
+                    acc[ft * TT + tt][4 * a + 2 * b2] = r0;
+                    acc[ft * TT + tt][4 * a + 2 * b2 + 1] = r1;
                 }
             }
         }
@@ -472,17 +579,14 @@
     __builtin_amdgcn_sched_barrier(0);
     float P[TT][4][5];
     {
-        const float* rcL = p.rope + (long)L * kRopeRow + 16 * hh;
 #pragma unroll
         for (int hd = 0; hd < 4; ++hd) {
-            const float* bk = p.bias_k + (4 * w + hd) * kDH;
+            const uint32_t* kt = &stage.tab[0][((2 * w + hh) * 4 + hd) * 6];
             float kb[12];
 #pragma unroll
             for (int q = 0; q < 6; ++q) {
-                const int i = 6 * hh + q;
-                const float x1 = bk[i], x2 = bk[i + 12], c = rcL[q], sn = rcL[8 + q];
-                kb[2 * q] = bf16_lo(pack_bf16(x1 * c - x2 * sn, 0.f));
-                kb[2 * q + 1] = bf16_lo(pack_bf16(x2 * c + x1 * sn, 0.f));
+                kb[2 * q] = bf16_lo(kt[q]);
+                kb[2 * q + 1] = bf16_hi(kt[q]);
             }
 #pragma unroll
             for (int tt = 0; tt < TT; ++tt) {
@@ -499,13 +603,21 @@
                     qf[2 * q] = bf16_lo(u);
                     qf[2 * q + 1] = bf16_hi(u);
                 }
-                float s[5] = {0.f, 0.f, 0.f, 0.f, 0.f};
+                dpp_fence(k);
+                float s[5];
+                s[0] = mul_dpp<0>(k[0], qf[0]);
+                s[1] = mul_dpp<1>(k[0], qf[0]);
+                s[2] = mul_dpp<2>(k[0], qf[0]);
+                s[3] = mul_dpp<3>(k[0], qf[0]);
+                s[4] = 0.f;
 #pragma unroll
                 for (int i = 0; i < 12; ++i) {
-                    s[0] += qf[i] * quad_bcast<0>(k[i]);
-                    s[1] += qf[i] * quad_bcast<1>(k[i]);
-                    s[2] += qf[i] * quad_bcast<2>(k[i]);
-                    s[3] += qf[i] * quad_bcast<3>(k[i]);
+                    if (i > 0) {
+                        s[0] = fmac_dpp<0>(s[0], k[i], qf[i]);
+                        s[1] = fmac_dpp<1>(s[1], k[i], qf[i]);
+                        s[2] = fmac_dpp<2>(s[2], k[i], qf[i]);
+                        s[3] = fmac_dpp<3>(s[3], k[i], qf[i]);
+                    }
                     s[4] += qf[i] * kb[i];
                 }
 #pragma unroll
@@ -542,10 +654,9 @@
         for (int i = 0; i < 20; ++i) qstash[w][i][lane] = pack_bf16(Pf[2 * i], Pf[2 * i + 1]);
     }
     __builtin_amdgcn_sched_barrier(0);
-    zero_acc<3 * TT>(acc);
-    wave_gemm<TT, 3, 24, true, HALF ? 4 : kAttn4VPF>(panel, kRowB, t0, 0, p.wv + (size_t)(3 * w) * 24 * 64 + lane, 24 * 64, acc);
+    wave_gemm<TT, 3, 24, true, HALF ? 4 : kAttn4VPF, true>(panel, kRowB, t0, 0, p.wv + (size_t)(3 * w) * 24 * 64 + lane, 24 * 64, acc);
     ATTN4_STAMP(7);
-    load_head_bias(p.bv, w, hh, bb);
+    load_head_bias(stage.bias[2], w, hh, bb);
     {
         float* Pf = &P[0][0][0];
 #pragma unroll
@@ -559,17 +670,28 @@
 #pragma unroll
     for (int hd = 0; hd < 4; ++hd) {
         const int head = 4 * w + hd;
+        const uint32_t* vt = &stage.tab[1][((2 * w + hh) * 4 + hd) * 6];
         float bvv[12];
 #pragma unroll
-        for (int i = 0; i < 12; ++i) bvv[i] = bf16_lo(pack_bf16(p.bias_v[head * kDH + 12 * hh + i], 0.f));
+        for (int q = 0; q < 6; ++q) {
+            bvv[2 * q] = bf16_lo(vt[q]);
+            bvv[2 * q + 1] = bf16_hi(vt[q]);
+        }
 #pragma unroll
         for (int tt = 0; tt < TT; ++tt) {
             float v[12], o[12];
             head_values<TT>(acc, tt, hd, bb[hd], v);
-#pragma unroll
-            for (int i = 0; i < 12; ++i)
-                o[i] = P[tt][hd][0] * quad_bcast<0>(v[i]) + P[tt][hd][1] * quad_bcast<1>(v[i]) +
-                       P[tt][hd][2] * quad_bcast<2>(v[i]) + P[tt][hd][3] * quad_bcast<3>(v[i]) + P[tt][hd][4] * bvv[i];
+            dpp_fence(v);
+#pragma unroll
+            for (int i = 0; i < 12; ++i) o[i] = mul_dpp<1>(v[i], P[tt][hd][1]);
+#pragma unroll
+            for (int i = 0; i < 12; ++i) o[i] = fmac_dpp<0>(o[i], v[i], P[tt][hd][0]);
+#pragma unroll
+            for (int i = 0; i < 12; ++i) o[i] = fmac_dpp<2>(o[i], v[i], P[tt][hd][2]);
+#pragma unroll
+            for (int i = 0; i < 12; ++i) o[i] = fmac_dpp<3>(o[i], v[i], P[tt][hd][3]);
+#pragma unroll
+            for (int i = 0; i < 12; ++i) o[i] = __builtin_fmaf(P[tt][hd][4], bvv[i], o[i]);
             if (PROJ) {
                 const bool ok = tok[tt] >= 0;
 #pragma unroll
@@ -588,8 +710,7 @@
     if (!PROJ) return;
     __syncthreads();
     ATTN4_STAMP(8);
-    zero_acc<3 * TT>(acc);
-    wave_gemm<TT, 3, 24, false>(panel, kRowB, t0, 0, p.wo + (size_t)(3 * w) * 24 * 64 + lane, 24 * 64, acc);
+    wave_gemm<TT, 3, 24, false, 4, true>(panel, kRowB, t0, 0, p.wo + (size_t)(3 * w) * 24 * 64 + lane, 24 * 64, acc);
     ATTN4_STAMP(9);
     __syncthreads();
     if constexpr (HALF) {
diff --git a/mdgen_amd/csrc/k_small.hip b/mdgen_amd/csrc/k_small.hip
--- a/mdgen_amd/csrc/k_small.hip
+++ b/mdgen_amd/csrc/k_small.hip
@@ -60,6 +60,21 @@
     }
     rope[(long)pos * kRopeRow + h * 16 + j] = c;
     rope[(long)pos * kRopeRow + h * 16 + 8 + j] = sn;
+}
+
+__global__ void k_l4_bias_table(const float* __restrict__ bias_k, const float* __restrict__ bias_v, const float* __restrict__ rope,
+                                uint32_t* __restrict__ tab) {
+    const int i = threadIdx.x;
+    if (i >= kL4Tab) return;
+    const int q = i % 6, g = i / 6, hd = g & 3, hh = (g >> 2) & 1, w = g >> 3;
+    const float* bk = bias_k + (4 * w + hd) * kDH;
+    const float* rcL = rope + 4 * kRopeRow + 16 * hh;
+    const int j = 6 * hh + q;
+    const float x1 = bk[j], x2 = bk[j + 12], c = rcL[q], sn = rcL[8 + q];
+    const float a = x2 * sn, b = x1 * sn;
+    tab[i] = pack_bf16(__builtin_fmaf(x1, c, -a), __builtin_fmaf(x2, c, b));
+    const float* bv = bias_v + (4 * w + hd) * kDH + 12 * hh;
+    tab[kL4Tab + i] = pack_bf16(bv[2 * q], bv[2 * q + 1]);
 }
 
 __global__ void k_gather_f32(const float* __restrict__ src, const int* __restrict__ idx, float scale,
@@ -586,6 +601,9 @@
 void launch_rope_table(float* rope, const float* inv_freq, int npos, hipStream_t s) {
     hipLaunchKernelGGL(k_rope_table, dim3((npos * 16 + 255) / 256), dim3(256), 0, s, rope, inv_freq, npos);
 }
+void launch_l4_bias_table(const float* bias_k, const float* bias_v, const float* rope, uint32_t* tab, hipStream_t s) {
+    hipLaunchKernelGGL(k_l4_bias_table, dim3(1), dim3(256), 0, s, bias_k, bias_v, rope, tab);
+}
 void launch_gather_f32(const float* src, const int* idx, float scale, float* dst, int n, hipStream_t s) {
     hipLaunchKernelGGL(k_gather_f32, dim3((n + 255) / 256), dim3(256), 0, s, src, idx, scale, dst, n);
 }
diff --git a/mdgen_amd/csrc/kernels.h b/mdgen_amd/csrc/kernels.h
--- a/mdgen_amd/csrc/kernels.h
+++ b/mdgen_amd/csrc/kernels.h
@@ -18,6 +18,7 @@
     uint32_t* vmask;
     int vmask_stride;
     const float *bias_k, *bias_v;
+    const uint32_t* l4tab;
     MaskMap mk;
     __bf16* obuf;
     float* h_rw;
@@ -402,6 +403,8 @@
                  const float* b2, float* silu_out, hipStream_t s);
 void launch_adaln(const float* st, int nrows, const float* w, const float* b, int nout, float* mod, hipStream_t s);
 void launch_rope_table(float* rope, const float* inv_freq, int npos, hipStream_t s);
+constexpr int kL4Tab = 192;
+void launch_l4_bias_table(const float* bias_k, const float* bias_v, const float* rope, uint32_t* tab, hipStream_t s);
 void launch_gather_f32(const float* src, const int* idx, float scale, float* dst, int n, hipStream_t s);
 void launch_pack_rows(const float* w, int ld, const int* rowmap, int nft, int ksteps, float scale, bf16x8* dst,
                       hipStream_t s, int kappa = 0, int part = 0);
diff --git a/mdgen_amd/csrc/panel.h b/mdgen_amd/csrc/panel.h
--- a/mdgen_amd/csrc/panel.h
+++ b/mdgen_amd/csrc/panel.h
@@ -15,13 +15,14 @@
     return *reinterpret_cast<const bf16x8*>(panel + panel_off(row, ks * 32 + (lane >> 5) * 16, rowb));
 }
 
-template <int TT, int FT, int KSTEPS, bool TRANS, int PF = 4>
+template <int TT, int FT, int KSTEPS, bool TRANS, int PF = 4, bool ZC = false>
 __device__ __forceinline__ void wave_gemm(const unsigned char* panel, const int rowb, const int tile0, const int ks0,
                                           const bf16x8* __restrict__ wfrag, const int wtile_stride,
                                           f32x16* acc) {
     static_assert(PF < KSTEPS, "prefetch depth");
     bf16x8 wring[PF + 1][FT];
     bf16x8 aring[2][TT];
+    const f32x16 zero = {0.f, 0.f, 0.f, 0.f, 0.f, 0.f, 0.f, 0.f, 0.f, 0.f, 0.f, 0.f, 0.f, 0.f, 0.f, 0.f};
 #pragma unroll
     for (int p = 0; p < PF; ++p)
 #pragma unroll
@@ -47,11 +48,18 @@
             for (int f = 0; f < FT; ++f) {
                 if (TRANS)
                     acc[f * TT + t] = __builtin_amdgcn_mfma_f32_32x32x16_bf16(wring[ks % (PF + 1)][f], aring[ks & 1][t],
-                                                                             acc[f * TT + t], 0, 0, 0);
+                                                                             ZC && ks == 0 ? zero : acc[f * TT + t], 0, 0, 0);
                 else
                     acc[t * FT + f] = __builtin_amdgcn_mfma_f32_32x32x16_bf16(aring[ks & 1][t], wring[ks % (PF + 1)][f],
-                                                                             acc[t * FT + f], 0, 0, 0);
-            }
+                                                                             ZC && ks == 0 ? zero : acc[t * FT + f], 0, 0, 0);
+            }
+        if (ZC && ks == 0) {
+#pragma unroll
+            for (int t = 0; t < TT; ++t)
+#pragma unroll
+                for (int f = 0; f < FT; ++f)
+                    asm volatile("" : "+v"(acc[TRANS ? f * TT + t : t * FT + f]) : "v"(wring[0][f]), "v"(aring[0][t]));
+        }
         __builtin_amdgcn_sched_barrier(0);
     }
 }
```
